# asmekal/ubdvss

Measured on AMD Instinct MI355X. Metric: images/sec (512x512) fwd+CCL, higher is better.
Workload: dtype f32; 1 GPU; configs[1]: batch=32 512x512x3 fp32 forward + CCL postprocess per GPU (stripe-textured rectangle images, random-init weights); batch_per_gpu=32, parallelism=replicas x1, no collective

## Files before the change

### ubdvss_amd/csrc/api.hip

```cpp
#include <stdarg.h>
#include <stddef.h>
#include <stdlib.h>
#include <string.h>
#include <thread>
#include "common.h"

static thread_local char g_err[512] = "";

void ubd_set_error(const char *fmt, ...)
{
    va_list ap;
    va_start(ap, fmt);
    vsnprintf(g_err, sizeof(g_err), fmt, ap);
    va_end(ap);
}

extern "C" const char *ubd_last_error(void) { return g_err; }
extern "C" int ubd_abi_version(void) { return UBD_ABI_VERSION; }
#ifndef UBD_BUILD_ID
#define UBD_BUILD_ID "unknown"
#endif
extern "C" int ubd_host_memcpy_mt(void *dst, const void *src, size_t n, int threads)
{
    if (threads < 1) threads = 1;
    if (threads > 16) threads = 16;
    if (n < ((size_t)1 << 20)) threads = 1;
    const size_t piece = ((n + threads - 1) / threads + 4095) & ~(size_t)4095;
    std::thread th[16];
    int started = 0;
    size_t done_to = n < piece ? n : piece;
    for (int t = 1; t < threads; ++t) {
        const size_t a = (size_t)t * piece;
        if (a >= n) break;
        const size_t len = n - a < piece ? n - a : piece;
        try {
            th[started] = std::thread([=] { memcpy((char *)dst + a, (const char *)src + a, len); });
            ++started;
        } catch (...) {
            memcpy((char *)dst + a, (const char *)src + a, n - a);
            break;
        }
    }
    memcpy(dst, src, done_to);
    for (int t = 0; t < started; ++t) th[t].join();
    return 0;
}
extern "C" const char *ubd_build_id(void) { return UBD_BUILD_ID; }

#ifdef UBD_STAMPS
static struct { const char *kernel; ubd_stamp_buf buf; int sel0, sel1; } g_stamps[] = {
    {"stem23"}, {"stem123"}, {"wino"}, {"wino6"}, {"sep123_16"}, {"dilconv16s"}, {"sepb16"}, {"sep_bwd"}, {"dil_wgrad16"}, {"postprocess"}, {"loss"},
};
extern "C" int ubd_debug_set_stamps(const char *kernel, void *buf, size_t capacity_words, int sel0, int sel1)
{
    for (auto &e : g_stamps)
        if (kernel && strcmp(kernel, e.kernel) == 0) {
            e.buf = {(unsigned long long *)buf, buf ? capacity_words : 0};
            e.sel0 = sel0; e.sel1 = sel1;
            return 0;
        }
    UBD_REQUIRE(false, "ubd_debug_set_stamps: no kernel family named %s", kernel ? kernel : "(null)");
}
ubd_stamp_buf ubd_stamps_for(const char *kernel, int sel0, int sel1)
{
    for (const auto &e : g_stamps)
        if (strcmp(kernel, e.kernel) == 0) return e.sel0 == sel0 && e.sel1 == sel1 ? e.buf : ubd_stamp_buf{nullptr, 0};
    return {nullptr, 0};
}
#endif

static const char ANY[] = "", NUMBER[] = "#";
struct env_switch { const char *name; size_t field; const char *value; int set; };
#define SW(name, field, value, set) {name, offsetof(ubd_handle, field), value, set}
static const env_switch ENV_SWITCHES[] = {
    SW("UBD_DILCONV", use_wino, "direct", 0), SW("UBD_DILCONV", wino_x6, "direct", 0), SW("UBD_DILCONV", wino_x6, "wino32", 0),
    SW("UBD_WINO6_LAYOUT", wino6_natural, "natural", 1),
    SW("UBD_STEM", fuse_stem, "fused", UBD_STEM_FUSED23), SW("UBD_STEM", fuse_force, "fused", 1),
    SW("UBD_STEM", fuse_stem, "fused123", UBD_STEM_FUSED123), SW("UBD_STEM", fuse_force, "fused123", 1),
    SW("UBD_STEM", fuse_stem, "unfused", UBD_STEM_SEPARATE),
    SW("UBD_TEST_NUM_CUS", num_cus, NUMBER, 0),
    SW("UBD_DILBWD", split_dilbwd, "split", 1), SW("UBD_DILBWD", no_pair_dilbwd, "pair8", 1),
    SW("UBD_SEPBWD", split_sepbwd32, "split", 1),
    SW("UBD_STEM16", split_stem16, "split", 1), SW("UBD_STEM16", split_stem16, "fused12", 2),
    SW("UBD_PP_GLOBAL", pp_global, ANY, 1), SW("UBD_PP_SPLIT", pp_split, ANY, 1), SW("UBD_PP_POISON", pp_poison, ANY, 1),
    SW("UBD_PP_SERIAL_TAIL", pp_serial_tail, ANY, 1), SW("UBD_PP_THREADS_512", pp_threads_512, ANY, 1),
    SW("UBD_HEADBWD", split_headbwd, "split", 1),
    SW("UBD_SEPB16_X", sepb_x_regs, "regs", 1),
    SW("UBD_REDUCE", chain_reduce, "batched", 0),
    SW("UBD_LOSS", loss_chain, "chain", 1),
    SW("UBD_DILCONV16", direct_dil16, "direct", 1),
};
#undef SW

extern "C" int ubd_create(const ubd_config *cfg, ubd_handle **out)
{
    UBD_REQUIRE(cfg && out, "ubd_create: null argument");
    UBD_REQUIRE(cfg->c_in == 1 || cfg->c_in == 3, "ubd_create: c_in must be 1 (grey) or 3, got %d", cfg->c_in);
    UBD_REQUIRE(cfg->n_classes >= 0 && cfg->n_classes <= UBD_MAX_CLASSES, "ubd_create: n_classes %d out of range [0,%d]", cfg->n_classes, UBD_MAX_CLASSES);
    UBD_REQUIRE(cfg->dtype == UBD_F32 || cfg->dtype == UBD_BF16 || cfg->dtype == UBD_F16, "ubd_create: bad dtype %d", cfg->dtype);
    int ndev = 0;
    hipError_t e = hipGetDeviceCount(&ndev);
    UBD_REQUIRE(e == hipSuccess && ndev > 0, "ubd_create: no HIP device visible (%s); this library has no CPU fallback", hipGetErrorString(e));
    int dev = 0;
    UBD_CHECK_HIP(hipGetDevice(&dev));
    hipDeviceProp_t prop;
    UBD_CHECK_HIP(hipGetDeviceProperties(&prop, dev));
    UBD_REQUIRE(strncmp(prop.gcnArchName, "gfx950", 6) == 0, "ubd_create: device arch %s is not gfx950; this library is built for MI355X only", prop.gcnArchName);

    ubd_handle *h = (ubd_handle *)calloc(1, sizeof(ubd_handle));
    UBD_REQUIRE(h, "ubd_create: out of host memory");
    h->cfg = *cfg;
    h->k_out = 1 + cfg->n_classes;
    h->num_cus = prop.multiProcessorCount;
    h->use_wino = h->wino_x6 = h->chain_reduce = 1;
    h->fuse_stem = cfg->fml_compatible != 0 ? UBD_STEM_FUSED123 : UBD_STEM_SEPARATE;
    for (const env_switch &sw : ENV_SWITCHES) {
        const char *e = getenv(sw.name);
        if (!e) continue;
        int *field = (int *)((char *)h + sw.field);
        if (sw.value == NUMBER) { if (atoi(e) > 0) *field = atoi(e); }
        else if (sw.value == ANY || strcmp(e, sw.value) == 0) *field = sw.set;
    }
    { const char *s = getenv("UBD_STEM"); if (s && strcmp(s, "cold123") == 0 && cfg->fml_compatible != 0) { h->fuse_stem = UBD_STEM_COLD123; h->fuse_force = 1; } }
    size_t off = 0;
    int cin = cfg->c_in;
    for (int s = 0; s < 3; ++s) {
        h->off_sep_dw[s] = off; off += (size_t)9 * cin;
        h->off_sep_pw[s] = off; off += (size_t)cin * UBD_C;
        h->off_sep_b[s] = off;  off += UBD_C;
        cin = UBD_C;
    }
    for (int k = 0; k < UBD_NUM_DIL; ++k) {
        h->off_dil_k[k] = off; off += (size_t)9 * UBD_C * UBD_C;
        h->off_dil_b[k] = off; off += UBD_C;
    }
    h->off_head_k = off; off += (size_t)UBD_C * h->k_out;
    h->off_head_b = off; off += h->k_out;
    h->n_params = off;
    *out = h;
    return 0;
}

extern "C" void ubd_destroy(ubd_handle *h)
{
    if (h && h->comm) ubd_comm_destroy(h);
    free(h);
}

extern "C" size_t ubd_param_count(const ubd_handle *h) { return h ? h->n_params : 0; }
extern "C" int ubd_num_cus(const ubd_handle *h) { return h ? h->num_cus : 0; }
```

### ubdvss_amd/csrc/common.h

```cpp
#pragma once
#include <hip/hip_runtime.h>
#include <stdint.h>
#include <stdio.h>
#include <string.h>
#include <type_traits>
#include "../../include/ubd.h"
#include "stem_plan.h"
#include "stamps.h"

#define UBD_C 24
#define UBD_NUM_DIL 6

struct ubd_comm;
struct ubd_handle {
    ubd_config cfg;
    ubd_comm *comm;
    int k_out;
    size_t off_sep_dw[3], off_sep_pw[3], off_sep_b[3];
    size_t off_dil_k[UBD_NUM_DIL], off_dil_b[UBD_NUM_DIL];
    size_t off_head_k, off_head_b;
    size_t n_params;
    int num_cus;
    int pp_lds_attr_set;
    int fuse_force;
    int split_headbwd;
    int no_pair_dilbwd;
    int split_dilbwd;
    int split_stem16;
    int pp_global, pp_split, pp_poison, pp_serial_tail, pp_threads_512;
    int sepb_x_regs;
    int split_sepbwd32;
    int chain_reduce;
    int direct_dil16;
    int fuse_stem;
    int use_wino;
    int loss_chain;
    int wino_x6;
    int wino6_natural;
};

static const int UBD_DILATIONS[UBD_NUM_DIL] = {1, 2, 4, 8, 16, 1};

#if defined(__HIPCC__)
__device__ __forceinline__ int ubd_xcd_tile(int L, int total)
{
    return (total & 7) == 0 ? (L & 7) * (total >> 3) + (L >> 3) : L;
}
#endif

#if defined(__HIPCC__)
__device__ __forceinline__ void ubd_glds16_at(const void *gsrc, unsigned lds_dst)
{
    unsigned keep;
    asm volatile("s_mov_b32 %0, m0\n\ts_mov_b32 m0, %2\n\ts_nop 0\n\tglobal_load_lds_dwordx4 %1, off\n\ts_mov_b32 m0, %0"
                 : "=&s"(keep) : "v"(gsrc), "s"(lds_dst) : "memory");
}
__device__ __forceinline__ void ubd_glds16_sbase(const void *base_uniform, unsigned voff, unsigned lds_dst)
{
    unsigned keep;
    asm volatile("s_mov_b32 %0, m0\n\ts_mov_b32 m0, %3\n\ts_nop 0\n\tglobal_load_lds_dwordx4 %1, %2\n\ts_mov_b32 m0, %0"
                 : "=&s"(keep) : "v"(voff), "s"(base_uniform), "s"(lds_dst) : "memory");
}
__device__ __forceinline__ void ubd_blds16(__amdgpu_buffer_rsrc_t rsrc, unsigned voff, unsigned lds_dst)
{
    unsigned keep;
    asm volatile("s_mov_b32 %0, m0\n\ts_mov_b32 m0, %3\n\ts_nop 0\n\tbuffer_load_dwordx4 %1, %2, 0 offen lds\n\ts_mov_b32 m0, %0"
                 : "=&s"(keep) : "v"(voff), "s"(rsrc), "s"(lds_dst) : "memory");
}
__device__ __forceinline__ void ubd_blds4(__amdgpu_buffer_rsrc_t rsrc, unsigned voff, unsigned lds_dst)
{
    unsigned keep;
    asm volatile("s_mov_b32 %0, m0\n\ts_mov_b32 m0, %3\n\ts_nop 0\n\tbuffer_load_dword %1, %2, 0 offen lds\n\ts_mov_b32 m0, %0"
                 : "=&s"(keep) : "v"(voff), "s"(rsrc), "s"(lds_dst) : "memory");
}
__device__ __forceinline__ float ubd_relu_cap(float x, float cap) { return __builtin_amdgcn_fmed3f(x, 0.f, cap); }
__device__ __forceinline__ unsigned ubd_lds_addr(const void *lds_generic)
{
    return (unsigned)__builtin_amdgcn_readfirstlane((int)(unsigned)(size_t)(__attribute__((address_space(3))) const char *)lds_generic);
}
__device__ __forceinline__ void ubd_glds16(const void *gsrc, const void *lds_generic) { ubd_glds16_at(gsrc, ubd_lds_addr(lds_generic)); }
#endif

#if defined(__HIPCC__)
template <int D, int NMAX> struct ubd_magic24 {
    static constexpr int find_sh()
    {
        for (int sh = 8; sh < 24; ++sh) {
            const long m = (1L << sh) / D + 1;
            if (m * NMAX >= (1L << 24)) continue;
            bool ok = true;
            for (long n = 0; n < NMAX && ok; ++n) ok = ((n * m) >> sh) == n / D;
            if (ok) return sh;
        }
        return -1;
    }
    static constexpr int sh = find_sh();
    static_assert(sh > 0, "no 24-bit magic number for this divisor / range");
    static constexpr unsigned m = (1u << sh) / D + 1;
};

__device__ __forceinline__ int ubd_mul24(int a, int b) { return __mul24(a, b); }
template <int D, int NMAX> __device__ __forceinline__ int ubd_div24(int n) { return (int)(__umul24((unsigned)n, ubd_magic24<D, NMAX>::m) >> ubd_magic24<D, NMAX>::sh); }
struct ubd_tile_decoder {
    unsigned tiles_x, tiles_y, mx, my, total;
    bool fast;
    __device__ __forceinline__ void init(int tx_, int ty_, int total_)
    {
        tiles_x = (unsigned)tx_; tiles_y = (unsigned)ty_; total = (unsigned)total_;
        mx = 0xFFFFFFFFu / tiles_x + 1u;
        my = 0xFFFFFFFFu / tiles_y + 1u;
        const unsigned dmax = tiles_x > tiles_y ? tiles_x : tiles_y;
        fast = (unsigned long long)total * dmax < 0x100000000ull;
    }
    __device__ __forceinline__ unsigned div_x(unsigned v) const { return fast ? (tiles_x == 1u ? v : __umulhi(v, mx)) : v / tiles_x; }
    __device__ __forceinline__ unsigned div_y(unsigned v) const { return fast ? (tiles_y == 1u ? v : __umulhi(v, my)) : v / tiles_y; }
    __device__ __forceinline__ void decode(int L, int &tx, int &ty, int &img) const
    {
        const unsigned tile = (unsigned)ubd_xcd_tile(L, (int)total);
        const unsigned r = div_x(tile);
        tx = (int)(tile - r * tiles_x);
        const unsigned im = div_y(r);
        ty = (int)(r - im * tiles_y);
        img = (int)im;
    }
};
#endif

void ubd_set_error(const char *fmt, ...);

#define UBD_CHECK_HIP(expr)                                                              \
    do {                                                                                 \
        hipError_t _e = (expr);                                                          \
        if (_e != hipSuccess) {                                                          \
            ubd_set_error("%s:%d: %s failed: %s", __FILE__, __LINE__, #expr,             \
                          hipGetErrorString(_e));                                        \
            return 1;                                                                    \
        }                                                                                \
    } while (0)

#define UBD_REQUIRE(cond, ...)                                                           \
    do {                                                                                 \
        if (!(cond)) {                                                                   \
            ubd_set_error(__VA_ARGS__);                                                  \
            return 2;                                                                    \
        }                                                                                \
    } while (0)

static inline size_t ubd_align_up(size_t v, size_t a) { return (v + a - 1) / a * a; }

static inline bool ubd_pixels_by_lds_dma(bool f32_in, float sub, float div, int H, int W, int c_in, size_t limit, const void *x)
{
    return f32_in && sub == 0.f && div == 1.f && (size_t)H * W * c_in * 4 < limit && ((uintptr_t)x & 15) == 0;
}
static inline bool ubd_head_in_epilogue(const ubd_handle *h) { return h->k_out == 1 && h->off_head_b == h->off_head_k + UBD_C; }
template <int V> using ubd_int = std::integral_constant<int, V>;
template <typename F> static inline void ubd_dispatch_bool(bool b, F f) { if (b) f(std::true_type{}); else f(std::false_type{}); }
template <typename F> static inline void ubd_dispatch_input(int c_in, bool u8, F f)
{
    if (c_in == 1) { if (u8) f(ubd_int<1>{}, ubd_int<1>{}); else f(ubd_int<1>{}, ubd_int<0>{}); }
    else { if (u8) f(ubd_int<3>{}, ubd_int<1>{}); else f(ubd_int<3>{}, ubd_int<0>{}); }
}

#define UBD_DIL_FRAG_FLOATS (9 * 6 * 2 * 64)
#define UBD_SEP_FRAG_FLOATS (6 * 2 * 64)
#define UBD_SEP_DW_FLOATS (9 * 6 * 64)
#define UBD_WINO_FRAG_FLOATS (16 * 6 * 64 * 2)
#define UBD_FWD_DIRECT_FLOATS (3 * (UBD_SEP_FRAG_FLOATS + UBD_SEP_DW_FLOATS) + UBD_NUM_DIL * UBD_DIL_FRAG_FLOATS)
#define UBD_WINO6_FRAG_U32 (16 * 2 * 3 * 64 * 4)
#define UBD_FWD_WINO6_OFF (UBD_FWD_DIRECT_FLOATS + UBD_NUM_DIL * UBD_WINO_FRAG_FLOATS)
#define UBD_FWD_FRAG_FLOATS (UBD_FWD_WINO6_OFF + UBD_NUM_DIL * UBD_WINO6_FRAG_U32)

struct ubd_fwd_layout {
    size_t off_tickets;
    size_t off_wfrag;
    size_t off_a1, off_a2;
    size_t off_b[2];
    size_t off_acts[7];
    size_t total;
};

bool ubd_comm_fused(const ubd_handle *h);
bool ubd_comm_global_loss(const ubd_handle *h);
int ubd_comm_rank(const ubd_handle *h);
enum { UBD_RED_F64 = 0, UBD_RED_I32 = 1, UBD_RED_U32 = 2 };
int ubd_comm_allreduce_raw(ubd_handle *h, void *buf, size_t count, int kind, hipStream_t st);
int ubd_comm_allgather_u32(ubd_handle *h, const unsigned *send_one, unsigned *recv_world, hipStream_t st);
extern "C" int ubd_comm_world(const ubd_handle *h);
int ubd_comm_begin_tail(ubd_handle *h, float *grads, hipStream_t st);
int ubd_comm_finish(ubd_handle *h, float *grads, hipStream_t st);
void ubd_fwd_layout_compute(const ubd_handle *h, int n, int H, int W, int training, ubd_fwd_layout *L);
struct pp_lds_args;
int ubd_forward_impl(ubd_handle *h, const float *params, const void *images, int in_dtype, int preprocessing,
                     int n, int H, int W, float *logits, char *ws, const ubd_fwd_layout &L, hipStream_t st, bool inference = false,
                     const pp_lds_args *pp_job = nullptr);
int ubd_pp_fill_job(ubd_handle *hd, const float *logits, int n, int map_h, int map_w, float logit_threshold, int scale, float min_area,
                    int32_t *binary_map, int32_t *quads, int32_t *classes, int32_t *counts, int cap, void *workspace,
                    size_t workspace_bytes, int threads, pp_lds_args *job);
void ubd_launch_dilconv(const ubd_handle *h, int epi, const float *frag, const float *aux, int dilation,
                        const float *in, float *out, int n, int H4, int W4, hipStream_t st);
int ubd_grid_for(long waves_needed, int num_cus, int waves_per_block, int blocks_per_cu);
int ubd_loss_impl(const float *logits, int k_out, const int32_t *y_true, long npix, float *loss, float *dlogits,
                  char *ws, hipStream_t st, ubd_handle *h = nullptr, bool prezeroed = false);
size_t ubd_loss_zero_bytes(void);
extern "C" size_t ubd_loss_workspace_bytes(const ubd_handle *h, int n, int map_h, int map_w);
void ubd_launch_pack_wino(const ubd_handle *h, const float *params, float *out, int transpose, hipStream_t st);
void ubd_launch_dilconv_wino(const ubd_handle *h, int epi, const float *frag, const void *aux, int aux_dtype, int dilation,
                             const float *in, float *out, int n, int H4, int W4, hipStream_t st, const float *head = nullptr);
void ubd_launch_pack_wino6(const ubd_handle *h, const float *params, unsigned *out, hipStream_t st);
void ubd_launch_dilconv_wino6(const ubd_handle *h, int epi, const unsigned *frag, const float *bias, int dilation,
                              const float *in, float *out, int n, int H4, int W4, hipStream_t st, const float *head = nullptr,
                              int lay_in = 1, int lay_out = 1);
void ubd_launch_pack_direct(const ubd_handle *h, const float *params, float *wfrag, hipStream_t st);
size_t ubd_forward16_workspace_bytes(int n, int H, int W);
int ubd_pack16_workspace(ubd_handle *h, const float *params, char *ws, size_t ws_bytes, hipStream_t st);
int ubd_forward16(ubd_handle *h, const float *params, const void *images, int in_dtype, int preprocessing, int n, int H, int W,
                  float *logits, char *ws, size_t ws_bytes, hipStream_t st);
#define UBD_SEP16_READY_U32 (2 * 10 * 64 * 4)
#define UBD_DIL16_FRAG_U32 (7 * 2 * 64 * 4)
void ubd_launch_dilconv16(const ubd_handle *h, int epi, const unsigned *frag, const float *bias, const void *mask, int d,
                          const void *in, void *out, int n, int H4, int W4, hipStream_t st, float *logits3 = nullptr);
void ubd_launch_pack16(const ubd_handle *h, const float *params, unsigned *out, int transpose, hipStream_t st);
struct ubd_fwd16_layout { size_t off_wfrag32, off_wfrag16, off_a1, off_a2, off_acts[7], total; };
void ubd_fwd16_layout_compute(int n, int H, int W, int training, ubd_fwd16_layout *L);
int ubd_forward16_layout(ubd_handle *h, const float *params, const void *images, int in_dtype, int preprocessing, int n, int H,
                         int W, float *logits, char *ws, const ubd_fwd16_layout &L, hipStream_t st, bool inference = false);
```

### ubdvss_amd/csrc/forward.hip

```cpp
#include "common.h"

typedef float f32x4 __attribute__((ext_vector_type(4)));
typedef float f32x2 __attribute__((ext_vector_type(2)));
typedef unsigned int u32x4 __attribute__((ext_vector_type(4)));
typedef unsigned int u32x2 __attribute__((ext_vector_type(2)));

#include "pack.h"
__global__ void pack_weights_kernel(const float *__restrict__ params, float *__restrict__ wfrag, pack_args a)
{
    pack_weights_body(params, wfrag, a, (int)(blockIdx.x * blockDim.x + threadIdx.x), (int)(gridDim.x * blockDim.x));
}

__device__ __forceinline__ void store_tile_relu(float *__restrict__ y, size_t row_base_elems, int x0, int ow,
                                                int lane, f32x4 acc0, f32x4 acc1, float b0, float b1)
{
    const int co = lane & 15, q = lane >> 4;
    const unsigned long long rp = (unsigned long long)(y + (row_base_elems + (size_t)x0) * UBD_C);
    const unsigned rlo = (unsigned)__builtin_amdgcn_readfirstlane((int)(unsigned)rp);
    const unsigned rhi = (unsigned)__builtin_amdgcn_readfirstlane((int)(unsigned)(rp >> 32));
    float *rowp = (float *)(((unsigned long long)rhi << 32) | rlo);
    int npx = ow - x0 < 16 ? ow - x0 : 16;
    npx = npx < 0 ? 0 : npx;
    const unsigned bytes = (unsigned)__builtin_amdgcn_readfirstlane(npx * UBD_C * 4);
    __amdgpu_buffer_rsrc_t rs = __builtin_amdgcn_make_buffer_rsrc((void *)rowp, 0, (int)bytes, 0x00020000);
    const unsigned base = (unsigned)(4 * q) * (UBD_C * 4u) + (unsigned)co * 4u;
    const unsigned base1 = co < 8 ? base + 64u : 0x40000000u;
#pragma unroll
    for (int r = 0; r < 4; ++r) {
        __builtin_amdgcn_raw_buffer_store_b32(__builtin_bit_cast(unsigned, fmaxf(acc0[r] + b0, 0.f)), rs, (int)(base + r * 96u), 0, 0);
        __builtin_amdgcn_raw_buffer_store_b32(__builtin_bit_cast(unsigned, fmaxf(acc1[r] + b1, 0.f)), rs, (int)(base1 + r * 96u), 0, 0);
    }
}

__device__ __forceinline__ void store_tile_relu_t(float *__restrict__ y, size_t row_base_elems, int x0, int ow,
                                                  int lane, f32x4 acc0, f32x4 acc1, f32x4 bA, f32x4 bB)
{
    const int i = lane & 15, q = lane >> 4;
    const unsigned long long rp = (unsigned long long)(y + (row_base_elems + (size_t)x0) * UBD_C);
    const unsigned rlo = (unsigned)__builtin_amdgcn_readfirstlane((int)(unsigned)rp);
    const unsigned rhi = (unsigned)__builtin_amdgcn_readfirstlane((int)(unsigned)(rp >> 32));
    float *rowp = (float *)(((unsigned long long)rhi << 32) | rlo);
    int npx = ow - x0 < 16 ? ow - x0 : 16;
    npx = npx < 0 ? 0 : npx;
    const unsigned bytes = (unsigned)__builtin_amdgcn_readfirstlane(npx * UBD_C * 4);
    __amdgpu_buffer_rsrc_t rs = __builtin_amdgcn_make_buffer_rsrc((void *)rowp, 0, (int)bytes, 0x00020000);
    const unsigned base = (unsigned)i * (UBD_C * 4u) + 16u * (unsigned)q;
    const unsigned base1 = q < 2 ? base + 64u : 0x40000000u;
    f32x4 o0, o1;
#pragma unroll
    for (int r = 0; r < 4; ++r) { o0[r] = fmaxf(acc0[r] + bA[r], 0.f); o1[r] = fmaxf(acc1[r] + bB[r], 0.f); }
    __builtin_amdgcn_raw_buffer_store_b128(__builtin_bit_cast(u32x4, o0), rs, (int)base, 0, 0);
    __builtin_amdgcn_raw_buffer_store_b128(__builtin_bit_cast(u32x4, o1), rs, (int)base1, 0, 0);
}

__device__ __forceinline__ void store_tile_relu_nb(float *__restrict__ y, size_t row_base_elems, int x0, int ow,
                                                   int lane, f32x4 acc0, f32x4 acc1, bool drop = false ,
                                                   int l2p = 0)
{
    const int i = lane & 15, q = lane >> 4;
    const unsigned long long rp = (unsigned long long)(y + row_base_elems * UBD_C);
    const unsigned rlo = (unsigned)__builtin_amdgcn_readfirstlane((int)(unsigned)rp);
    const unsigned rhi = (unsigned)__builtin_amdgcn_readfirstlane((int)(unsigned)(rp >> 32));
    float *rowp = (float *)(((unsigned long long)rhi << 32) | rlo);
    const unsigned bytes = (unsigned)__builtin_amdgcn_readfirstlane(ow * UBD_C * 4);
    __amdgpu_buffer_rsrc_t rs = __builtin_amdgcn_make_buffer_rsrc((void *)rowp, 0, (int)bytes, 0x00020000);
    const int x = x0 + i, r = x & ((1 << l2p) - 1), wr = ow & ((1 << l2p) - 1);
    const int pos = r * (ow >> l2p) + (r < wr ? r : wr) + (x >> l2p);
    const unsigned base = (drop || x >= ow) ? 0x40000000u : (unsigned)pos * (UBD_C * 4u) + 16u * (unsigned)q;
    const unsigned base1 = (q < 2 && !drop) ? base + 64u : 0x40000000u;
    const float cap = __builtin_inff();
    f32x4 o0, o1;
#pragma unroll
    for (int r = 0; r < 4; ++r) { o0[r] = ubd_relu_cap(acc0[r], cap); o1[r] = ubd_relu_cap(acc1[r], cap); }
    __builtin_amdgcn_raw_buffer_store_b128(__builtin_bit_cast(u32x4, o0), rs, (int)base, 0, 0);
    __builtin_amdgcn_raw_buffer_store_b128(__builtin_bit_cast(u32x4, o1), rs, (int)base1, 0, 0);
}

__device__ __forceinline__ void store_tile_masked(float *__restrict__ y, const float (&mk)[8],
                                                  size_t row_base_elems, int x0, int ow, int lane, f32x4 acc0, f32x4 acc1)
{
    const int co = lane & 15, q = lane >> 4;
#pragma unroll
    for (int r = 0; r < 4; ++r) {
        int px = x0 + 4 * q + r;
        if (px < ow) {
            const size_t e = (row_base_elems + (size_t)px) * UBD_C;
            y[e + co] = mk[r] > 0.f ? acc0[r] : 0.f;
            if (co < 8) y[e + 16 + co] = mk[4 + r] > 0.f ? acc1[r] : 0.f;
        }
    }
}

template <int CIN, int STRIDE> struct sep_cfg {
    static constexpr int TH = (CIN == UBD_C) ? (STRIDE == 2 ? 4 : 8) : 16;
    static constexpr int PH = (TH - 1) * STRIDE + 3;
    static constexpr int PW = 15 * STRIDE + 3;
    static constexpr int PS = CIN;
    static constexpr int CHUNKS = (CIN == UBD_C) ? PH * PW * 6 : 0;
    static constexpr int ELEMS = PH * PW * CIN;
    static constexpr int BUF_FLOATS = (CIN == UBD_C) ? (CHUNKS + 255) / 256 * 256 * 4 : (ELEMS + 3) / 4 * 4;
    static constexpr int STAGE_REGS = (CIN == UBD_C) ? 1 : (ELEMS + 255) / 256;
};

template <int CIN, int STRIDE, int IN_U8>
__global__ __launch_bounds__(256, (CIN == UBD_C) ? (STRIDE == 1 ? 3 : 2) : 5) void sepconv_kernel(const void *__restrict__ xin, float *__restrict__ y,
                                                      const float *__restrict__ frag,
                                                      const float *__restrict__ bias, int n, int H, int W, int OH,
                                                      int OW, int pad_lo, float pre_sub, float pre_div)
{
    using C = sep_cfg<CIN, STRIDE>;
    constexpr int CPL = (CIN == UBD_C) ? 6 : 1;
    constexpr int NBUF = (CIN == UBD_C) ? 2 : 1;
    __shared__ __attribute__((aligned(16))) float patch_mem[NBUF * C::BUF_FLOATS];
    const int lane = threadIdx.x & 63, wid = __builtin_amdgcn_readfirstlane((int)(threadIdx.x >> 6));
    const int i = lane & 15, q = lane >> 4;
    const float *pwfrag = frag;
    const float *dwlane = frag + UBD_SEP_FRAG_FLOATS;

    const int tiles_x = (OW + 15) >> 4, tiles_y = (OH + C::TH - 1) / C::TH;
    const int total = n * tiles_y * tiles_x;

    float dwk[9][CPL];
    float pwf[CPL][2];
#pragma unroll
    for (int s = 0; s < CPL; ++s) {
        const int ch = (CIN == UBD_C) ? (s < 4 ? 4 * q + s : 16 + 2 * q + (s - 4)) : 0;
        const int src_lane = (CIN == UBD_C) ? 16 * (ch / 6) + i : lane, ss = (CIN == UBD_C) ? ch % 6 : s;
#pragma unroll
        for (int t = 0; t < 9; ++t) dwk[t][s] = dwlane[(t * 6 + ss) * 64 + src_lane];
        pwf[s][0] = pwfrag[(ss * 2 + 0) * 64 + src_lane];
        pwf[s][1] = pwfrag[(ss * 2 + 1) * 64 + src_lane];
    }
    const f32x4 bA = *(const f32x4 *)(bias + 4 * q);
    const f32x4 bB = q < 2 ? *(const f32x4 *)(bias + 16 + 4 * q) : f32x4{0.f, 0.f, 0.f, 0.f};
    const int cb = (q < CIN) ? q : 0;

    ubd_tile_decoder tdec;
    tdec.init(tiles_x, tiles_y, total);
    auto tile_coords = [&](int tile, int &img, int &oy0, int &ox0) {
        int tx, ty;
        tdec.decode(tile, tx, ty, img);
        oy0 = ty * C::TH; ox0 = tx * 16;
    };
    constexpr int ROUNDS = (CIN == UBD_C) ? (C::CHUNKS + 255) / 256 : 1;
    int dma_rel[ROUNDS];
    if constexpr (CIN == UBD_C) {
#pragma unroll
        for (int rd = 0; rd < ROUNDS; ++rd) {
            int c = rd * 256 + wid * 64 + lane;
            c = c < C::CHUNKS ? c : C::CHUNKS - 1;
            const int pix = c / 6, sp = c - pix * 6;
            const int pr = pix / C::PW, pc = pix - pr * C::PW;
            int part = sp + 3 * ((pc >> 3) & 1);
            part = part >= 6 ? part - 6 : part;
            dma_rel[rd] = ((pr * W + pc) * UBD_C + part * 4) * 4;
        }
    }
    auto dma_tile = [&](int tile, float *buf) {
        int img, oy0, ox0;
        tile_coords(tile, img, oy0, ox0);
        const int ix0 = ox0 * STRIDE - pad_lo, iy0 = oy0 * STRIDE - pad_lo;
        const char *src = (const char *)xin;
        const bool interior = (iy0 >= 0) && (ix0 >= 0) && (iy0 + C::PH <= H) && (ix0 + C::PW <= W);
        if (interior) {
            const char *origin = src + (((size_t)img * H + iy0) * W + ix0) * (UBD_C * sizeof(float));
#pragma unroll
            for (int rd = 0; rd < ROUNDS; ++rd)
                __builtin_amdgcn_global_load_lds((const __attribute__((address_space(1))) void *)(origin + dma_rel[rd]),
                                                 (__attribute__((address_space(3))) void *)(buf + (rd * 256 + wid * 64) * 4), 16, 0, 0);
            return;
        }
        __amdgpu_buffer_rsrc_t rsrc = __builtin_amdgcn_make_buffer_rsrc((void *)(src + (size_t)img * H * W * (UBD_C * sizeof(float))), 0,
                                                                        (int)((unsigned)H * W * (unsigned)(UBD_C * sizeof(float))), 0x00020000);
#pragma unroll
        for (int rd = 0; rd < ROUNDS; ++rd) {
            const int cbase = rd * 256 + wid * 64;
            int c = cbase + lane;
            c = c < C::CHUNKS ? c : C::CHUNKS - 1;
            const int pix = c / 6, sp = c - pix * 6;
            const int pr = pix / C::PW, pc = pix - pr * C::PW;
            int part = sp + 3 * ((pc >> 3) & 1);
            part = part >= 6 ? part - 6 : part;
            const int gy = iy0 + pr, gx = ix0 + pc;
            const unsigned off = (unsigned)gx < (unsigned)W ? (unsigned)(((gy * W + gx) * UBD_C + part * 4) * (int)sizeof(float)) : 0x80000000u;
            __builtin_amdgcn_raw_ptr_buffer_load_lds(rsrc, (__attribute__((address_space(3))) void *)(buf + cbase * 4), 16, (int)off, 0, 0, 0);
        }
    };
    int ld_rel[C::STAGE_REGS];
    if constexpr (CIN != UBD_C) {
#pragma unroll
        for (int k = 0; k < C::STAGE_REGS; ++k) {
            int e = k * 256 + threadIdx.x;
            e = e < C::ELEMS ? e : C::ELEMS - 1;
            const int pix = e / CIN, ch = e - pix * CIN;
            const int pr = pix / C::PW, pc = pix - pr * C::PW;
            ld_rel[k] = (pr * W + pc) * CIN + ch;
        }
    }
    auto load_regs = [&](int tile, unsigned (&st)[C::STAGE_REGS]) {
        int img, oy0, ox0;
        tile_coords(tile, img, oy0, ox0);
        const int ix0 = ox0 * STRIDE - pad_lo, iy0 = oy0 * STRIDE - pad_lo;
        const bool interior = (iy0 >= 0) && (ix0 >= 0) && (iy0 + C::PH <= H) && (ix0 + C::PW <= W);
        if (interior) {
            const size_t origin = (((size_t)img * H + iy0) * W + ix0) * CIN;
#pragma unroll
            for (int k = 0; k < C::STAGE_REGS; ++k) {
                if constexpr (IN_U8) st[k] = ((const unsigned char *)xin)[origin + ld_rel[k]];
                else st[k] = ((const unsigned *)xin)[origin + ld_rel[k]];
            }
            return;
        }
        const int WC = W * CIN;
        const unsigned char *img8 = (const unsigned char *)xin + (size_t)img * H * WC * ((IN_U8) ? 1 : 4);
#pragma unroll
        for (int k = 0; k < C::STAGE_REGS; ++k) {
            int e = k * 256 + threadIdx.x;
            e = e < C::ELEMS ? e : C::ELEMS - 1;
            const int pr = e / (C::PW * CIN), pf = e - pr * (C::PW * CIN);
            const int gy = min(max(iy0 + pr, 0), H - 1), gf = min(max(ix0 * CIN + pf, 0), WC - 1);
            const unsigned off = (unsigned)(gy * WC + gf);
            if constexpr (IN_U8) st[k] = img8[off];
            else st[k] = ((const unsigned *)img8)[off];
        }
#pragma unroll
        for (int k = 0; k < C::STAGE_REGS; ++k) {
            int e = k * 256 + threadIdx.x;
            e = e < C::ELEMS ? e : C::ELEMS - 1;
            const int pr = e / (C::PW * CIN), pf = e - pr * (C::PW * CIN);
            const bool inside = (unsigned)(iy0 + pr) < (unsigned)H && (unsigned)(ix0 * CIN + pf) < (unsigned)WC;
            st[k] = inside ? st[k] : ((IN_U8) ? 0x100u : __builtin_bit_cast(unsigned, pre_sub));
        }
    };

    int tile = blockIdx.x;
    if (tile >= total) return;
    unsigned stage[C::STAGE_REGS];
    if constexpr (CIN == UBD_C) dma_tile(tile, patch_mem);
    else load_regs(tile, stage);

    for (int it = 0;; ++it) {
        float *patch = patch_mem + ((CIN == UBD_C) ? (it & 1) * C::BUF_FLOATS : 0);
        int img, oy0, ox0;
        tile_coords(tile, img, oy0, ox0);
        const int nxt = tile + gridDim.x;
        const bool has_next = (CIN == UBD_C) && nxt < total;
        if constexpr (CIN == UBD_C) {
            constexpr int NSTORE = (C::TH / 4) * 2;
            if (it == 0) asm volatile("s_waitcnt vmcnt(0)" ::: "memory");
            else if constexpr (NSTORE == 8) asm volatile("s_waitcnt vmcnt(8)" ::: "memory");
            else if constexpr (NSTORE == 4) asm volatile("s_waitcnt vmcnt(4)" ::: "memory");
            else { static_assert(NSTORE == 2, "counted vmcnt"); asm volatile("s_waitcnt vmcnt(2)" ::: "memory"); }
            __builtin_amdgcn_s_barrier();
            if (has_next) dma_tile(nxt, patch_mem + ((it + 1) & 1) * C::BUF_FLOATS);
        } else {
            __builtin_amdgcn_s_barrier();
#pragma unroll
            for (int k = 0; k < C::STAGE_REGS; ++k) {
                const int e = k * 256 + threadIdx.x;
                if (e < C::ELEMS) {
                    if constexpr (IN_U8) patch[e] = stage[k] > 255u ? 0.f : ((float)stage[k] - pre_sub) / pre_div;
                    else patch[e] = (__builtin_bit_cast(float, stage[k]) - pre_sub) / pre_div;
                }
            }
            __builtin_amdgcn_s_waitcnt(0xC07F);
            __builtin_amdgcn_s_barrier();
            if (has_next) load_regs(nxt, stage);
        }

        if constexpr (CIN == UBD_C && STRIDE == 1) {
            constexpr int RW = C::TH / 4;
            const int rb = wid * RW;
            float dwv[RW][6];
#pragma unroll
            for (int o = 0; o < RW; ++o)
#pragma unroll
                for (int s = 0; s < 6; ++s) dwv[o][s] = 0.f;
#pragma unroll
            for (int yy = 0; yy < RW + 2; ++yy) {
                f32x4 v4[3];
                f32x2 v2[3];
#pragma unroll
                for (int kx = 0; kx < 3; ++kx) {
                    const int pcol = i + kx;
                    const float *p = patch + ((rb + yy) * C::PW + pcol) * C::PS;
                    const int rot = 3 * ((pcol >> 3) & 1);
                    int s4 = q + rot, s2 = 4 + (q >> 1) + rot;
                    s4 = s4 >= 6 ? s4 - 6 : s4; s2 = s2 >= 6 ? s2 - 6 : s2;
                    v4[kx] = *(const f32x4 *)(p + 4 * s4);
                    v2[kx] = *(const f32x2 *)(p + 4 * s2 + 2 * (q & 1));
                }
#pragma unroll
                for (int o = 0; o < RW; ++o) {
                    const int ky = yy - o;
                    if (ky < 0 || ky > 2) continue;
#pragma unroll
                    for (int kx = 0; kx < 3; ++kx) {
                        const int t = ky * 3 + kx;
                        dwv[o][0] = fmaf(v4[kx][0], dwk[t][0], dwv[o][0]);
                        dwv[o][1] = fmaf(v4[kx][1], dwk[t][1], dwv[o][1]);
                        dwv[o][2] = fmaf(v4[kx][2], dwk[t][2], dwv[o][2]);
                        dwv[o][3] = fmaf(v4[kx][3], dwk[t][3], dwv[o][3]);
                        dwv[o][4] = fmaf(v2[kx][0], dwk[t][4], dwv[o][4]);
                        dwv[o][5] = fmaf(v2[kx][1], dwk[t][5], dwv[o][5]);
                    }
                }
                if (yy >= 2) {
                    const int o = yy - 2, oy = oy0 + rb + o;
                    f32x4 acc0 = {0.f, 0.f, 0.f, 0.f}, acc1 = {0.f, 0.f, 0.f, 0.f};
#pragma unroll
                    for (int s = 0; s < 6; ++s) {
                        acc0 = __builtin_amdgcn_mfma_f32_16x16x4f32(pwf[s][0], dwv[o][s], acc0, 0, 0, 0);
                        acc1 = __builtin_amdgcn_mfma_f32_16x16x4f32(pwf[s][1], dwv[o][s], acc1, 0, 0, 0);
                    }
                    store_tile_relu_t(y, ((size_t)img * OH + oy) * OW, ox0, oy < OH ? OW : 0, lane, acc0, acc1, bA, bB);
                }
            }
        } else {
        for (int r = wid; r < C::TH; r += 4) {
            const int oy = oy0 + r;
            float dwv[CPL];
#pragma unroll
            for (int s = 0; s < CPL; ++s) dwv[s] = 0.f;
#pragma unroll
            for (int ky = 0; ky < 3; ++ky) {
#pragma unroll
                for (int kx = 0; kx < 3; ++kx) {
                    const int pcol = i * STRIDE + kx;
                    const float *p = patch + ((r * STRIDE + ky) * C::PW + pcol) * C::PS;
                    const int t = ky * 3 + kx;
                    if constexpr (CIN == UBD_C) {
                        const int rot = 3 * ((pcol >> 3) & 1);
                        int s4 = q + rot, s2 = 4 + (q >> 1) + rot;
                        s4 = s4 >= 6 ? s4 - 6 : s4; s2 = s2 >= 6 ? s2 - 6 : s2;
                        const f32x4 v4 = *(const f32x4 *)(p + 4 * s4);
                        const f32x2 v2 = *(const f32x2 *)(p + 4 * s2 + 2 * (q & 1));
                        dwv[0] = fmaf(v4[0], dwk[t][0], dwv[0]);
                        dwv[1] = fmaf(v4[1], dwk[t][1], dwv[1]);
                        dwv[2] = fmaf(v4[2], dwk[t][2], dwv[2]);
                        dwv[3] = fmaf(v4[3], dwk[t][3], dwv[3]);
                        dwv[4] = fmaf(v2[0], dwk[t][4], dwv[4]);
                        dwv[5] = fmaf(v2[1], dwk[t][5], dwv[5]);
                    } else {
                        dwv[0] = fmaf(p[cb], dwk[t][0], dwv[0]);
                    }
                }
            }
            f32x4 acc0 = {0.f, 0.f, 0.f, 0.f}, acc1 = {0.f, 0.f, 0.f, 0.f};
#pragma unroll
            for (int s = 0; s < CPL; ++s) {
                acc0 = __builtin_amdgcn_mfma_f32_16x16x4f32(pwf[s][0], dwv[s], acc0, 0, 0, 0);
                acc1 = __builtin_amdgcn_mfma_f32_16x16x4f32(pwf[s][1], dwv[s], acc1, 0, 0, 0);
            }
            store_tile_relu_t(y, ((size_t)img * OH + oy) * OW, ox0, oy < OH ? OW : 0, lane, acc0, acc1, bA, bB);
        }
        }
        if (!has_next) break;
        tile = nxt;
    }
}

#include "pp_lds.h"
#include "stem23.h"
#include "stem123.h"

struct a_frags {
    f32x4 v4[9];
    f32x2 v2[9];
};

__device__ __forceinline__ void dil_load(a_frags &a, __amdgpu_buffer_rsrc_t rsrc, unsigned oob, int tile,
                                         int tiles_x, int h, int w, int d, int lane)
{
    const int i = lane & 15, q = lane >> 4;
    const int xt = (int)((unsigned)tile % (unsigned)tiles_x);
    const int rowid = (int)((unsigned)tile / (unsigned)tiles_x);
    const int yy = (int)((unsigned)rowid % (unsigned)h);
    const int px = xt * 16 + i;
#pragma unroll
    for (int ky = 0; ky < 3; ++ky) {
        const int iy = yy + (ky - 1) * d;
        const bool rok = (iy >= 0) && (iy < h);
#pragma unroll
        for (int kx = 0; kx < 3; ++kx) {
            const int ix = px + (kx - 1) * d;
            const bool ok = rok && (ix >= 0) && (ix < w);
            const unsigned byte_off = (unsigned)((rowid + (ky - 1) * d) * w + ix) * (unsigned)(UBD_C * 4);
            const unsigned o4 = ok ? byte_off + 16u * q : oob;
            const unsigned o2 = ok ? byte_off + 64u + 8u * q : oob;
            u32x4 r4 = __builtin_amdgcn_raw_buffer_load_b128(rsrc, (int)o4, 0, 0);
            u32x2 r2 = __builtin_amdgcn_raw_buffer_load_b64(rsrc, (int)o2, 0, 0);
            a.v4[ky * 3 + kx] = __builtin_bit_cast(f32x4, r4);
            a.v2[ky * 3 + kx] = __builtin_bit_cast(f32x2, r2);
        }
    }
}

template <int EPI>
__global__ __launch_bounds__(256, 2) void dilconv_f32_kernel(const float *__restrict__ x, float *__restrict__ y,
                                                             const float *__restrict__ wfrag,
                                                             const float *__restrict__ bias, int n, int h, int w,
                                                             int d, unsigned in_bytes)
{
    const int lane = threadIdx.x & 63;
    const int i = lane & 15;
    float wr[9][6][2];
#pragma unroll
    for (int t = 0; t < 9; ++t)
#pragma unroll
        for (int j = 0; j < 6; ++j) {
            wr[t][j][0] = wfrag[((t * 6 + j) * 2 + 0) * 64 + lane];
            wr[t][j][1] = wfrag[((t * 6 + j) * 2 + 1) * 64 + lane];
        }
    float b0 = 0.f, b1 = 0.f;
    if constexpr (EPI == 0) { b0 = bias[i]; b1 = (i < 8) ? bias[16 + i] : 0.f; }

    const int tiles_x = (w + 15) >> 4;
    const int total = n * h * tiles_x;
    const int xcd = blockIdx.x & 7;
    const int nblk_x = (gridDim.x + 7 - xcd) >> 3;
    const int chunk = (total + 7) >> 3;
    const int t_begin = xcd * chunk;
    const int t_end = (t_begin + chunk < total) ? t_begin + chunk : total;
    const int stride = nblk_x * 4;
    int tile = t_begin + (int)(blockIdx.x >> 3) * 4 + __builtin_amdgcn_readfirstlane((int)(threadIdx.x >> 6));
    if (tile >= t_end) return;

    __amdgpu_buffer_rsrc_t rsrc = __builtin_amdgcn_make_buffer_rsrc((void *)x, 0, (int)in_bytes, 0x00020000);
    const unsigned oob = in_bytes;

    auto compute_store = [&](const a_frags &a, int tl) {
        f32x4 acc0 = {0.f, 0.f, 0.f, 0.f}, acc1 = {0.f, 0.f, 0.f, 0.f};
        float mk[8];
        if constexpr (EPI == 1) {
            const int co = lane & 15, q = lane >> 4;
            const int xt0 = (int)((unsigned)tl % (unsigned)tiles_x);
            const int rid = (int)((unsigned)tl / (unsigned)tiles_x);
#pragma unroll
            for (int r = 0; r < 4; ++r) {
                const int opx = xt0 * 16 + 4 * q + r;
                const size_t e = ((size_t)rid * w + (size_t)(opx < w ? opx : 0)) * UBD_C;
                mk[r] = bias[e + co];
                mk[4 + r] = bias[e + 16 + (co & 7)];
            }
        }
#pragma unroll
        for (int t = 0; t < 9; ++t) {
#pragma unroll
            for (int j = 0; j < 4; ++j) {
                acc0 = __builtin_amdgcn_mfma_f32_16x16x4f32(a.v4[t][j], wr[t][j][0], acc0, 0, 0, 0);
                acc1 = __builtin_amdgcn_mfma_f32_16x16x4f32(a.v4[t][j], wr[t][j][1], acc1, 0, 0, 0);
            }
#pragma unroll
            for (int j = 0; j < 2; ++j) {
                acc0 = __builtin_amdgcn_mfma_f32_16x16x4f32(a.v2[t][j], wr[t][4 + j][0], acc0, 0, 0, 0);
                acc1 = __builtin_amdgcn_mfma_f32_16x16x4f32(a.v2[t][j], wr[t][4 + j][1], acc1, 0, 0, 0);
            }
        }
        const int xt = (int)((unsigned)tl % (unsigned)tiles_x);
        const int rowid = (int)((unsigned)tl / (unsigned)tiles_x);
        if constexpr (EPI == 0) store_tile_relu(y, (size_t)rowid * w, xt * 16, w, lane, acc0, acc1, b0, b1);
        else store_tile_masked(y, mk, (size_t)rowid * w, xt * 16, w, lane, acc0, acc1);
    };

    a_frags A0, A1;
    const int t_last = t_end - 1;
    dil_load(A0, rsrc, oob, tile, tiles_x, h, w, d, lane);
    for (;;) {
        int nxt = tile + stride;
        dil_load(A1, rsrc, oob, nxt < t_last ? nxt : t_last, tiles_x, h, w, d, lane);
        compute_store(A0, tile);
        tile = nxt;
        if (tile >= t_end) break;
        nxt = tile + stride;
        dil_load(A0, rsrc, oob, nxt < t_last ? nxt : t_last, tiles_x, h, w, d, lane);
        compute_store(A1, tile);
        tile = nxt;
        if (tile >= t_end) break;
    }
}

__global__ __launch_bounds__(256) void head_kernel(const float *__restrict__ x, float *__restrict__ logits,
                                                   const float *__restrict__ hk, const float *__restrict__ hb,
                                                   long npix, int k_out)
{
    __shared__ float s_k[UBD_C * (UBD_MAX_CLASSES + 1)];
    __shared__ float s_b[UBD_MAX_CLASSES + 1];
    for (int t = threadIdx.x; t < UBD_C * k_out; t += blockDim.x) s_k[t] = hk[t];
    for (int t = threadIdx.x; t < k_out; t += blockDim.x) s_b[t] = hb[t];
    __syncthreads();
    for (long p = (long)blockIdx.x * blockDim.x + threadIdx.x; p < npix; p += (long)gridDim.x * blockDim.x) {
        const f32x4 *px = (const f32x4 *)(x + p * UBD_C);
        float v[UBD_C];
#pragma unroll
        for (int c4 = 0; c4 < 6; ++c4) {
            f32x4 t = px[c4];
            v[c4 * 4 + 0] = t[0]; v[c4 * 4 + 1] = t[1]; v[c4 * 4 + 2] = t[2]; v[c4 * 4 + 3] = t[3];
        }
        for (int ko = 0; ko < k_out; ++ko) {
            float acc = 0.f;
#pragma unroll
            for (int c = 0; c < UBD_C; ++c) acc = fmaf(v[c], s_k[c * k_out + ko], acc);
            logits[p * k_out + ko] = acc + s_b[ko];
        }
    }
}

static size_t act_bytes(const ubd_handle *, long n, long hh, long ww) { return (size_t)(n * hh * ww) * UBD_C * sizeof(float); }

void ubd_fwd_layout_compute(const ubd_handle *h, int n, int H, int W, int training, ubd_fwd_layout *L)
{
    const size_t wf = (size_t)UBD_FWD_FRAG_FLOATS * sizeof(float);
    size_t off = 0;
    L->off_wfrag = off; off += ubd_align_up(wf, 256);
    L->off_tickets = off; off += 256;
    const size_t a = ubd_align_up(act_bytes(h, n, H / 2, W / 2), 256);
    const size_t b = ubd_align_up(act_bytes(h, n, H / 4, W / 4), 256);
    L->off_a1 = off; off += a;
    L->off_a2 = off; off += a;
    if (training) {
        for (int k = 0; k < 7; ++k) { L->off_acts[k] = off; off += b; }
        L->off_b[0] = L->off_acts[0]; L->off_b[1] = L->off_acts[1];
    } else {
        L->off_b[0] = off; off += b;
        L->off_b[1] = off; off += b;
        for (int k = 0; k < 7; ++k) L->off_acts[k] = L->off_b[k & 1];
    }
    L->total = off;
}

extern "C" size_t ubd_forward_workspace_bytes(const ubd_handle *h, int n, int height, int width)
{
    if (h && h->cfg.dtype != UBD_F32) return ubd_forward16_workspace_bytes(n, height, width);
    ubd_fwd_layout L;
    ubd_fwd_layout_compute(h, n, height, width, 0, &L);
    return L.total;
}

int ubd_grid_for(long waves_needed, int num_cus, int waves_per_block, int blocks_per_cu)
{
    long blocks = (waves_needed + waves_per_block - 1) / waves_per_block;
    long cap = (long)num_cus * blocks_per_cu;
    if (blocks > cap) blocks = cap;
    if (blocks < 1) blocks = 1;
    return (int)blocks;
}

template <int CIN, int STRIDE>
static void launch_sep(const ubd_handle *h, const void *x, int in_u8, float *y, const float *frag, const float *bias,
                       int n, int H, int W, int OH, int OW, int pad_lo, float sc, float sh, hipStream_t st)
{
    const int th = sep_cfg<CIN, STRIDE>::TH;
    const int tiles = n * ((OH + th - 1) / th) * ((OW + 15) / 16);
    const int per_cu = (CIN == UBD_C) ? (STRIDE == 1 ? 3 : 2) : 5;
    int grid = h->num_cus * per_cu;
    if (grid > tiles || CIN != UBD_C) grid = tiles;
    ubd_dispatch_bool(in_u8 != 0, [&](auto u8) {
        hipLaunchKernelGGL((sepconv_kernel<CIN, STRIDE, decltype(u8)::value>), dim3(grid), dim3(256), 0, st, x, y, frag, bias, n, H, W, OH, OW, pad_lo, sc, sh);
    });
}

void ubd_launch_pack_direct(const ubd_handle *h, const float *params, float *wfrag, hipStream_t st)
{
    pack_args pa;
    for (int s = 0; s < 3; ++s) { pa.off_sep_dw[s] = h->off_sep_dw[s]; pa.off_sep_pw[s] = h->off_sep_pw[s]; }
    for (int k = 0; k < UBD_NUM_DIL; ++k) pa.off_dil_k[k] = h->off_dil_k[k];
    pa.c_in = h->cfg.c_in;
    hipLaunchKernelGGL(pack_weights_kernel, dim3(64), dim3(256), 0, st, params, wfrag, pa);
}

static void launch_pack(const ubd_handle *h, const float *params, float *wfrag, hipStream_t st)
{
    ubd_launch_pack_direct(h, params, wfrag, st);
    if (h->use_wino) ubd_launch_pack_wino(h, params, wfrag + UBD_FWD_DIRECT_FLOATS, 0, st);
    if (h->wino_x6) ubd_launch_pack_wino6(h, params, (unsigned *)(wfrag + UBD_FWD_WINO6_OFF), st);
}

void ubd_launch_dilconv(const ubd_handle *h, int epi, const float *frag, const float *aux, int dilation,
                        const float *in, float *out, int n, int H4, int W4, hipStream_t st)
{
    const unsigned in_bytes = (unsigned)((size_t)n * H4 * W4 * UBD_C * 4);
    const long tiles = (long)n * H4 * ((W4 + 15) / 16);
    int grid = ubd_grid_for(tiles, h->num_cus, 4, 2);
    grid = (grid + 7) / 8 * 8;
    if (epi == 0)
        hipLaunchKernelGGL(dilconv_f32_kernel<0>, dim3(grid), dim3(256), 0, st, in, out, frag, aux, n, H4, W4, dilation, in_bytes);
    else
        hipLaunchKernelGGL(dilconv_f32_kernel<1>, dim3(grid), dim3(256), 0, st, in, out, frag, aux, n, H4, W4, dilation, in_bytes);
}

static void launch_dil(const ubd_handle *h, const float *params, const float *wfrag, int k, const float *in, float *out,
                       int n, int H4, int W4, hipStream_t st, int lay_in = 1, int lay_out = 1)
{
    if (h->wino_x6) {
        ubd_launch_dilconv_wino6(h, 0, (const unsigned *)(wfrag + UBD_FWD_WINO6_OFF) + (size_t)k * UBD_WINO6_FRAG_U32, params + h->off_dil_b[k],
                                 UBD_DILATIONS[k], in, out, n, H4, W4, st, nullptr, lay_in, lay_out);
        return;
    }
    if (h->use_wino) {
        ubd_launch_dilconv_wino(h, 0, wfrag + UBD_FWD_DIRECT_FLOATS + (size_t)k * UBD_WINO_FRAG_FLOATS, params + h->off_dil_b[k], UBD_F32,
                                UBD_DILATIONS[k], in, out, n, H4, W4, st);
        return;
    }
    const int per_sep = UBD_SEP_FRAG_FLOATS + UBD_SEP_DW_FLOATS;
    const float *dfrag = wfrag + 3 * per_sep;
    ubd_launch_dilconv(h, 0, dfrag + (size_t)k * UBD_DIL_FRAG_FLOATS, params + h->off_dil_b[k], UBD_DILATIONS[k], in, out, n, H4, W4, st);
}

extern "C" int ubd_pack_weights(ubd_handle *h, const float *params, void *workspace, size_t workspace_bytes, void *stream)
{
    UBD_REQUIRE(h && params && workspace, "ubd_pack_weights: null argument");
    if (h->cfg.dtype != UBD_F32) return ubd_pack16_workspace(h, params, (char *)workspace, workspace_bytes, (hipStream_t)stream);
    ubd_fwd_layout L;
    ubd_fwd_layout_compute(h, 1, 4, 4, 0, &L);
    UBD_REQUIRE(workspace_bytes >= L.off_a1, "ubd_pack_weights: workspace too small");
    launch_pack(h, params, (float *)((char *)workspace + L.off_wfrag), (hipStream_t)stream);
    UBD_CHECK_HIP(hipMemsetAsync((char *)workspace + L.off_tickets, 0, 256, (hipStream_t)stream));
    UBD_CHECK_HIP(hipGetLastError());
    return 0;
}

extern "C" int ubd_dilated_layer(ubd_handle *h, const float *params, int layer, const void *in, void *out, int n,
                                 int map_h, int map_w, const void *workspace, void *stream)
{
    UBD_REQUIRE(h && params && in && out && workspace, "ubd_dilated_layer: null argument");
    UBD_REQUIRE(layer >= 0 && layer < UBD_NUM_DIL, "ubd_dilated_layer: layer %d out of range", layer);
    UBD_REQUIRE(h->cfg.dtype == UBD_F32, "ubd_dilated_layer: only UBD_F32 in this build");
    UBD_REQUIRE((size_t)n * map_h * map_w * UBD_C * 4 <= (1ull << 30), "ubd_dilated_layer: tensor too large (activation bytes must not exceed 2^30)");
    launch_dil(h, params, (const float *)workspace, layer, (const float *)in, (float *)out, n, map_h, map_w, (hipStream_t)stream);
    UBD_CHECK_HIP(hipGetLastError());
    return 0;
}

static int check_forward_input(int n, int H, int W, int in_dtype)
{
    UBD_REQUIRE(n > 0 && H > 0 && W > 0 && (H % 4) == 0 && (W % 4) == 0, "ubd_forward: height and width must be positive multiples of 4 (got %d x %d)", H, W);
    UBD_REQUIRE((in_dtype & ~UBD_IN_PREPACKED) == UBD_IN_F32 || (in_dtype & ~UBD_IN_PREPACKED) == UBD_IN_U8, "ubd_forward: bad in_dtype %d", in_dtype);
    return 0;
}

template <bool COLD>
static void launch_stem123(const ubd_handle *h, const float *params, const void *images, bool u8, float *a3, const float *sf0, const float *sf1,
                           const float *sf2, int n, int H, int W, float sc, float sh, long units, int *ticket, const pp_lds_args *job, int a3_l2p,
                           hipStream_t st)
{
    const int H2 = H / 2, W2 = W / 2, H4 = H / 4, W4 = W / 4;
    const int grid = units < h->num_cus ? (int)units : h->num_cus;
    pp_lds_args pj;
    memset(&pj, 0, sizeof(pj));
    if (job) pj = *job;
    const float *b0 = params + h->off_sep_b[0], *b1 = params + h->off_sep_b[1], *b2 = params + h->off_sep_b[2];
    const bool plain = ubd_pixels_by_lds_dma(!u8, sc, sh, H, W, h->cfg.c_in, 1ull << 30, images);
    ubd_dispatch_input(h->cfg.c_in, u8, [&](auto cin, auto in_u8) {
        auto launch = [&](auto pl) {
            hipLaunchKernelGGL((stem123_kernel<decltype(cin)::value, decltype(in_u8)::value, decltype(pl)::value, COLD>), dim3(grid), dim3(s23_cfg::NT), 0, st,
                               images, a3, sf0, b0, sf1, b1, sf2, b2, n, H, W, H2, W2, H4, W4, sc, sh, ticket, pj, a3_l2p
                               UBD_STAMP_ARG(COLD ? "" : "stem123"));
        };
        if constexpr (decltype(in_u8)::value == 0) { if (plain) return launch(ubd_int<1>{}); }
        launch(ubd_int<0>{});
    });
}

int ubd_forward_impl(ubd_handle *h, const float *params, const void *images, int in_dtype, int preprocessing,
                     int n, int H, int W, float *logits, char *ws, const ubd_fwd_layout &L, hipStream_t st, bool inference,
                     const pp_lds_args *pp_job)
{
    UBD_REQUIRE(h->cfg.dtype == UBD_F32, "ubd_forward: only UBD_F32 activations are implemented in this build");
    const bool prepacked = (in_dtype & UBD_IN_PREPACKED) != 0;
    in_dtype &= ~UBD_IN_PREPACKED;
    if (int rc = check_forward_input(n, H, W, in_dtype)) return rc;
    UBD_REQUIRE(!(in_dtype == UBD_IN_U8 && h->cfg.c_in == UBD_C), "ubd_forward: u8 input needs c_in 1 or 3");
    const int H2 = H / 2, W2 = W / 2, H4 = H / 4, W4 = W / 4;
    UBD_REQUIRE((size_t)n * H4 * W4 * UBD_C * 4 <= (1ull << 30), "ubd_forward: batch too large for 32-bit buffer offsets; split the batch");
    float *wfrag = (float *)(ws + L.off_wfrag);
    float *a1 = (float *)(ws + L.off_a1), *a2 = (float *)(ws + L.off_a2);

    if (!prepacked) {
        launch_pack(h, params, wfrag, st);
        UBD_CHECK_HIP(hipMemsetAsync(ws + L.off_tickets, 0, 256, st));
    }

    const int per_sep = UBD_SEP_FRAG_FLOATS + UBD_SEP_DW_FLOATS;
    const float *sf0 = wfrag, *sf1 = wfrag + per_sep, *sf2 = wfrag + 2 * per_sep;
    const int pad_s2 = h->cfg.fml_compatible ? 1 : 0;
    float sc = 0.f, sh = 1.f;
    if (preprocessing == UBD_PRE_MOBILENET) { sc = 127.5f; sh = 127.5f; }
    const int u8 = in_dtype == UBD_IN_U8;
    float *cur = (float *)(ws + L.off_acts[0]);
    static_assert(UBD_STEM_STRIP_ROWS == s23_cfg::TH3, "stem_plan.h counts the strips the stem kernels walk");
    const ubd_stem_plan plan = ubd_plan_stem(h->fuse_stem, h->fuse_force != 0, h->cfg.fml_compatible != 0, h->num_cus, n, H, inference, pp_job != nullptr);
    UBD_REQUIRE(!plan.job_without_strips, "ubd_forward: a postprocess job needs the fused stem kernel (internal error)");
    const bool one_kernel = plan.form == UBD_STEM_FORM_STRIPS || plan.form == UBD_STEM_FORM_COLD;
    static const int phase_lay[UBD_NUM_DIL + 1] = {2, 4, 1, 1, 1, 2, 1};
    const bool phase_major = h->wino_x6 && !h->wino6_natural && one_kernel;
    const int a3_l2p = phase_major ? 1 : 0;
    int *ticket = (int *)(ws + L.off_tickets);
    if (plan.form == UBD_STEM_FORM_COLD)
        launch_stem123<true>(h, params, images, u8, cur, sf0, sf1, sf2, n, H, W, sc, sh, plan.strips * (W4 <= 16 ? 1 : 1 + (W4 - 16 + 14) / 15),
                             ticket, nullptr, a3_l2p, st);
    else if (plan.form == UBD_STEM_FORM_STRIPS)
        launch_stem123<false>(h, params, images, u8, cur, sf0, sf1, sf2, n, H, W, sc, sh, plan.strips, ticket, pp_job, a3_l2p, st);
    else if (h->cfg.c_in == 1)
        launch_sep<1, 2>(h, images, u8, a1, sf0, params + h->off_sep_b[0], n, H, W, H2, W2, pad_s2, sc, sh, st);
    else
        launch_sep<3, 2>(h, images, u8, a1, sf0, params + h->off_sep_b[0], n, H, W, H2, W2, pad_s2, sc, sh, st);
    if (plan.form == UBD_STEM_FORM_L1_STEM23) {
        const int grid = plan.strips < h->num_cus ? (int)plan.strips : h->num_cus;
        ubd_dispatch_bool(pad_s2 != 0, [&](auto pad) {
            hipLaunchKernelGGL(stem23_kernel<decltype(pad)::value>, dim3(grid), dim3(s23_cfg::NT), 0, st, a1, cur, sf1, params + h->off_sep_b[1], sf2,
                               params + h->off_sep_b[2], n, H2, W2, H4, W4, pad_s2 UBD_STAMP_ARG("stem23"));
        });
    } else if (plan.form == UBD_STEM_FORM_SEPARATE) {
        launch_sep<UBD_C, 1>(h, a1, 0, a2, sf1, params + h->off_sep_b[1], n, H2, W2, H2, W2, 1, 0.f, 1.f, st);
        launch_sep<UBD_C, 2>(h, a2, 0, cur, sf2, params + h->off_sep_b[2], n, H2, W2, H4, W4, pad_s2, 0.f, 1.f, st);
    }

    const bool fuse_head = inference && h->use_wino && ubd_head_in_epilogue(h);
    for (int k = 0; k < UBD_NUM_DIL; ++k) {
        float *nxt = (float *)(ws + L.off_acts[k + 1]);
        if (fuse_head && k == UBD_NUM_DIL - 1) {
            if (h->wino_x6)
                ubd_launch_dilconv_wino6(h, 2, (const unsigned *)(wfrag + UBD_FWD_WINO6_OFF) + (size_t)k * UBD_WINO6_FRAG_U32, params + h->off_dil_b[k],
                                         UBD_DILATIONS[k], cur, logits, n, H4, W4, st, params + h->off_head_k, phase_major ? phase_lay[k] : 1, 1);
            else
                ubd_launch_dilconv_wino(h, 2, wfrag + UBD_FWD_DIRECT_FLOATS + (size_t)k * UBD_WINO_FRAG_FLOATS, params + h->off_dil_b[k], UBD_F32,
                                        UBD_DILATIONS[k], cur, logits, n, H4, W4, st, params + h->off_head_k);
            UBD_CHECK_HIP(hipGetLastError());
            return 0;
        }
        launch_dil(h, params, wfrag, k, cur, nxt, n, H4, W4, st, phase_major ? phase_lay[k] : 1, phase_major ? phase_lay[k + 1] : 1);
        cur = nxt;
    }
    const long npix = (long)n * H4 * W4;
    int hgrid = (int)((npix + 255) / 256);
    if (hgrid > h->num_cus * 8) hgrid = h->num_cus * 8;
    hipLaunchKernelGGL(head_kernel, dim3(hgrid), dim3(256), 0, st, cur, logits, params + h->off_head_k, params + h->off_head_b, npix, h->k_out);
    UBD_CHECK_HIP(hipGetLastError());
    return 0;
}

static int forward_f32(ubd_handle *h, const float *params, const void *images, int in_dtype, int preprocessing, int n, int H, int W, float *logits,
                       void *workspace, size_t workspace_bytes, void *stream, const pp_lds_args *pp_job)
{
    ubd_fwd_layout L;
    ubd_fwd_layout_compute(h, n, H, W, 0, &L);
    UBD_REQUIRE(workspace_bytes >= L.total, "ubd_forward: workspace too small (%zu < %zu)", workspace_bytes, L.total);
    return ubd_forward_impl(h, params, images, in_dtype, preprocessing, n, H, W, logits, (char *)workspace, L, (hipStream_t)stream, true, pp_job);
}

extern "C" int ubd_forward(ubd_handle *h, const float *params, const void *images, int in_dtype, int preprocessing,
                           int n, int height, int width, float *logits, void *workspace, size_t workspace_bytes,
                           void *stream)
{
    UBD_REQUIRE(h && params && images && logits && workspace, "ubd_forward: null argument");
    if (h->cfg.dtype != UBD_F32) {
        if (int rc = check_forward_input(n, height, width, in_dtype)) return rc;
        return ubd_forward16(h, params, images, in_dtype, preprocessing, n, height, width, logits, (char *)workspace, workspace_bytes, (hipStream_t)stream);
    }
    return forward_f32(h, params, images, in_dtype, preprocessing, n, height, width, logits, workspace, workspace_bytes, stream, nullptr);
}

extern "C" int ubd_forward_postprocess(ubd_handle *h, const float *params, const void *images, int in_dtype, int preprocessing,
                                       int n, int height, int width, float *logits, void *workspace, size_t workspace_bytes,
                                       const float *pp_logits, int pp_n, int pp_map_h, int pp_map_w, float logit_threshold, int scale,
                                       float min_area, int32_t *binary_map, int32_t *quads, int32_t *classes, int32_t *counts, int cap,
                                       void *pp_workspace, size_t pp_workspace_bytes, void *stream)
{
    UBD_REQUIRE(h && params && images && logits && workspace, "ubd_forward_postprocess: null argument");
    UBD_REQUIRE(pp_logits != logits, "ubd_forward_postprocess: the logits being postprocessed must not be the buffer this call writes");
    if (h->cfg.dtype == UBD_F32 && n > 0 && height > 0 && (height % 4) == 0 &&
        ubd_plan_stem(h->fuse_stem, h->fuse_force != 0, h->cfg.fml_compatible != 0, h->num_cus, n, height, true, true).form == UBD_STEM_FORM_STRIPS) {
        pp_lds_args job;
        const int fits = ubd_pp_fill_job(h, pp_logits, pp_n, pp_map_h, pp_map_w, logit_threshold, scale, min_area, binary_map, quads, classes,
                                         counts, cap, pp_workspace, pp_workspace_bytes,
                                         s23_cfg::NT, &job);
        if (fits < 0) return 1;
        if (fits == 1) return forward_f32(h, params, images, in_dtype, preprocessing, n, height, width, logits, workspace, workspace_bytes, stream, &job);
    }
    int rc = ubd_postprocess(h, pp_logits, pp_n, pp_map_h, pp_map_w, logit_threshold, scale, min_area, binary_map, quads, classes, counts, cap,
                             pp_workspace, pp_workspace_bytes, stream);
    if (rc) return rc;
    return ubd_forward(h, params, images, in_dtype, preprocessing, n, height, width, logits, workspace, workspace_bytes, stream);
}
```

### ubdvss_amd/csrc/stem123.h

```cpp
#pragma once
#include "split3.h"

__device__ __forceinline__ int s123_slot(int c, int col) { return c < 4 ? (c ^ ((col >> 2) & 1)) : 4 + ((c - 4) ^ ((col >> 3) & 1)); }

template <int CIN> struct s123_cfg {
    using B = s23_cfg;
    static constexpr int NT = B::NT, NW = B::NW;
    static constexpr int AC = B::LC + 1;
    static constexpr int XH = 2 * B::PH + 1, XW = 2 * AC + 1;
    static constexpr int XE = XH * XW * CIN;
    static constexpr int XREGS = (XE + NT - 1) / NT;
    static constexpr int XCH = ((XW + 1) * CIN + 3) / 4;
    static constexpr int XS = XCH * 4;
    static constexpr int XP_FLOATS = XH * XS;
    static constexpr int A1_FLOATS = B::PH * B::PW * UBD_C;
    static constexpr int NPIX = B::PH * AC;
    static constexpr int UNITS = (NPIX + 15) / 16;
    static constexpr int UPW = (UNITS + NW - 1) / NW;
    static constexpr int W1_FLOATS = 64 * 12 + 64 + 4;
    static constexpr int LUT_FLOATS = 256;
    static constexpr int PWS_U32 = 2 * 3 * 64 * 4;
    static constexpr int STEM_FLOATS = A1_FLOATS + B::L2_FLOATS + XP_FLOATS + 2 * PWS_U32 + B::W3DW_FLOATS + B::CARRY_FLOATS + W1_FLOATS + LUT_FLOATS;
    static constexpr int PP_FLOATS = (PP_LDS_MAX_BYTES + 3) / 4;
    static constexpr int SMEM_FLOATS = STEM_FLOATS > PP_FLOATS ? STEM_FLOATS : PP_FLOATS;
    static_assert(XCH <= 64 && (A1_FLOATS % 4) == 0 && (B::L2_FLOATS % 4) == 0, "patch rows are single 16-byte-aligned DMA pieces");
};

template <int CIN, int IN_U8, int PLAIN, bool COLD = false>
__global__ __launch_bounds__(s23_cfg::NT, 1) void stem123_kernel(const void *__restrict__ xin, float *__restrict__ y,
                                                                const float *__restrict__ frag1, const float *__restrict__ bias1,
                                                                const float *__restrict__ frag2, const float *__restrict__ bias2,
                                                                const float *__restrict__ frag3, const float *__restrict__ bias3,
                                                                int n, int H, int W, int H2, int W2, int H4, int W4,
                                                                float pre_sub, float pre_div, int *__restrict__ ticket, pp_lds_args pj,
                                                                int a3_l2p
                                                                UBD_STAMP_PARAM)
{
    using C = s23_cfg;
    using X = s123_cfg<CIN>;
    __shared__ __attribute__((aligned(16))) float smem[X::SMEM_FLOATS];
#define S123_BLOCK_STAMP(k) UBD_STAMP_RT(threadIdx.x == 0 && (k) < 32, (size_t)gridDim.x * 8 * 16 * 8 + (size_t)blockIdx.x * 32 + (k))
    S123_BLOCK_STAMP(0);
    if (pj.n > 0) {
        for (int im = (int)blockIdx.x; im < pj.n; im += (int)gridDim.x) {
            pp_image_lds<C::NT, true>((int *)smem, pj, im);
            __syncthreads();
        }
    }
    S123_BLOCK_STAMP(1);
    const int Dc = ((W4 + 15) >> 4) >= 3 ? 1 : 4 - ((W4 + 15) >> 4);
    const int njob = pj.n > 0 ? (pj.n < (int)gridDim.x ? pj.n : (int)gridDim.x) : 0;
    auto ticket_ls = [&](int k) { return k < njob * Dc ? k : k + ((int)gridDim.x - njob) * Dc; };
    int t0_early = 0;
    if (!COLD && threadIdx.x == 0 && (int)blockIdx.x < njob) t0_early = __hip_atomic_fetch_add(ticket, Dc, __ATOMIC_RELAXED, __HIP_MEMORY_SCOPE_AGENT);
    float *a1p = smem;
    float *l2 = a1p + X::A1_FLOATS;
    float *xp = l2 + C::L2_FLOATS;
    unsigned *pws = (unsigned *)(xp + X::XP_FLOATS);
    float *w3dw = (float *)(pws + 2 * X::PWS_U32);
    float *carry_buf = w3dw + C::W3DW_FLOATS;
    const int lane = threadIdx.x & 63, wid = __builtin_amdgcn_readfirstlane((int)(threadIdx.x >> 6));
    const int i = lane & 15, q = lane >> 4;

    float dwk2[9][6];
#pragma unroll
    for (int s = 0; s < 6; ++s) {
        const int ch = s < 4 ? 4 * q + s : 16 + 2 * q + (s - 4);
        const int src_lane = 16 * (ch / 6) + i, ss = ch % 6;
#pragma unroll
        for (int t = 0; t < 9; ++t) dwk2[t][s] = frag2[UBD_SEP_FRAG_FLOATS + (t * 6 + ss) * 64 + src_lane];
    }
    auto pw_split = [&](const unsigned *tab, f32x4 v4, f32x2 v2, f32x4 &acc0, f32x4 &acc1) {
        const u32x4 *w = (const u32x4 *)tab + lane;
        const f32x4 r4 = resid(v4), t4 = resid(r4);
        const f32x2 r2 = resid(v2), t2 = resid(r2);
        const u32x4 P1 = pack6(v4, v2), P2 = pack6(r4, r2), P3 = pack6(t4, t2);
        u32x4 U0 = w[2 * 64], U1 = w[5 * 64];
        acc0 = mfma16(U0, P1, acc0); acc1 = mfma16(U1, P1, acc1);
        U0 = w[1 * 64]; U1 = w[4 * 64];
        acc0 = mfma16(U0, P2, acc0); acc1 = mfma16(U1, P2, acc1);
        acc0 = mfma16(U0, P1, acc0); acc1 = mfma16(U1, P1, acc1);
        U0 = w[0]; U1 = w[3 * 64];
        acc0 = mfma16(U0, P3, acc0); acc1 = mfma16(U1, P3, acc1);
        acc0 = mfma16(U0, P2, acc0); acc1 = mfma16(U1, P2, acc1);
        acc0 = mfma16(U0, P1, acc0); acc1 = mfma16(U1, P1, acc1);
    };
    float *w1t = carry_buf + C::CARRY_FLOATS;
    float *bt = w1t + 64 * 12;
    const f32x4 z4 = {0.f, 0.f, 0.f, 0.f};
    const f32x4 b2A = *(const f32x4 *)(bias2 + 4 * q), b2B = q < 2 ? *(const f32x4 *)(bias2 + 16 + 4 * q) : z4;

    const int cold_kx = W4 <= 16 ? 1 : 1 + (W4 - 16 + 14) / 15;
    const int tiles_x = COLD ? 1 : (W4 + 15) >> 4, tiles_y = (H4 + C::TH3 - 1) / C::TH3;
    const int strips = COLD ? n * tiles_y * cold_kx : n * tiles_y;
    const int D = tiles_x >= 3 ? 1 : 4 - tiles_x;
    int *ring = (int *)(bt + 64);
    float *lut = bt + 64 + 4;
    struct tpos { int tx, ty, img, ord, ls; };
    auto strip_pos = [&](int ord, int tx) {
        tpos p;
        if constexpr (COLD) {
            const int ls = (int)blockIdx.x + ord * (int)gridDim.x;
            const int sidx = ubd_xcd_tile(ls < strips ? ls : strips - 1, strips);
            const int rowi = (int)((unsigned)sidx / (unsigned)cold_kx);
            p.tx = sidx - rowi * cold_kx;
            p.ty = (int)((unsigned)rowi % (unsigned)tiles_y);
            p.img = (int)((unsigned)rowi / (unsigned)tiles_y);
            p.ord = ord; p.ls = ls;
            return p;
        }
        const int ls = __builtin_amdgcn_readfirstlane(ring[ord & 3]);
        const int sidx = ubd_xcd_tile(ls < strips ? ls : strips - 1, strips);
        p.ty = (int)((unsigned)sidx % (unsigned)tiles_y);
        p.img = (int)((unsigned)sidx / (unsigned)tiles_y);
        p.tx = tx; p.ord = ord; p.ls = ls;
        return p;
    };
    auto advance = [&](tpos p) {
        if (!COLD && p.tx + 1 < tiles_x) { ++p.tx; return p; }
        return strip_pos(p.ord + 1, 0);
    };
    auto xo3 = [&](const tpos &p) { return (COLD ? 15 : 16) * p.tx; };

    unsigned xreg[X::XREGS];
    constexpr int RWF = X::XW * CIN;
    const int e0_row = (int)threadIdx.x / RWF, e0_col = (int)threadIdx.x - e0_row * RWF;
    auto tile_interior = [&](tpos p) {
        const int iy0 = 4 * p.ty * C::TH3 - 5, ix0 = 4 * xo3(p) - 3;
        return (iy0 >= 0) && (ix0 >= 0) && (iy0 + X::XH <= H) && (ix0 + X::XW <= W);
    };
    auto load_x = [&](tpos p) {
        const int iy0 = 4 * p.ty * C::TH3 - 5, fx0 = (4 * xo3(p) - 3) * CIN, WC = W * CIN;
        const unsigned char *img8 = (const unsigned char *)xin + (size_t)p.img * H * WC * (IN_U8 ? 1 : 4);
        const bool interior = tile_interior(p);
        int pr = e0_row, pcf = e0_col;
#pragma unroll
        for (int k = 0; k < X::XREGS; ++k) {
            int gy = iy0 + pr, gf = fx0 + pcf;
            if (!interior) { gy = min(max(gy, 0), H - 1); gf = min(max(gf, 0), WC - 1); }
            else if (k == X::XREGS - 1) gy = min(gy, H - 1);
            const unsigned off = (unsigned)__umul24(gy, WC) + (unsigned)gf;
            if constexpr (IN_U8) xreg[k] = img8[off];
            else xreg[k] = ((const unsigned *)img8)[off];
            pr += C::NT / RWF; pcf += C::NT % RWF;
            if (pcf >= RWF) { pcf -= RWF; ++pr; }
        }
    };
    auto fix_border = [&](tpos p) {
        const int iy0 = 4 * p.ty * C::TH3 - 5, fx0 = (4 * xo3(p) - 3) * CIN, WC = W * CIN;
        int pr = e0_row, pcf = e0_col;
#pragma unroll
        for (int k = 0; k < X::XREGS; ++k) {
            const bool inside = (unsigned)(iy0 + pr) < (unsigned)H && (unsigned)(fx0 + pcf) < (unsigned)WC;
            xreg[k] = inside ? xreg[k] : (IN_U8 ? 0x100u : __builtin_bit_cast(unsigned, pre_sub));
            pr += C::NT / RWF; pcf += C::NT % RWF;
            if (pcf >= RWF) { pcf -= RWF; ++pr; }
        }
    };

    const unsigned lds_xp = ubd_lds_addr(xp);
    auto dma_x = [&](tpos p) {
        const int iy0 = 4 * p.ty * C::TH3 - 5, fx0 = (4 * xo3(p) - 4) * CIN, WC = W * CIN;
        __amdgpu_buffer_rsrc_t rsrc = __builtin_amdgcn_make_buffer_rsrc((void *)((const char *)xin + (size_t)p.img * H * WC * 4), 0,
                                                                        (int)((unsigned)H * WC * 4u), 0x00020000);
        unsigned off0 = (unsigned)lane * 16u;
        off0 = (unsigned)(fx0 + 4 * lane) < (unsigned)WC ? off0 : 0x80000000u;
        if (lane < X::XCH) {
#pragma unroll
            for (int k = 0; k < (X::XH + C::NW - 1) / C::NW; ++k) {
                const int row = k * C::NW + wid;
                if (row >= X::XH) break;
                const int term = ((iy0 + row) * WC + fx0) * 4;
                ubd_blds16(rsrc, (unsigned)term + off0, lds_xp + (unsigned)(row * X::XS * 4));
            }
        }
    };

    constexpr int UPW = 4;
    int u_rc[UPW];
#pragma unroll
    for (int k = 0; k < UPW; ++k) {
        const int u = wid >= 4 ? (wid - 4) + 4 * k : (k < 2 ? 16 + wid + 4 * k : X::UNITS);
        const int p = u * 16 + i;
        const bool live = u < X::UNITS && p < X::NPIX;
        const int ar = (live ? p : 0) / X::AC, ac = (live ? p : 0) - ar * X::AC + 1;
        u_rc[k] = live ? ((ar << 8) | ac) : -1;
    }
    auto u_rc_tile = [&](int k) {
        int rc = u_rc[k];
        if constexpr (!PLAIN) asm volatile("" : "+v"(rc));
        return rc;
    };
    const int qc = q < CIN ? q : CIN - 1;
    const int half = wid & 1, rg = wid >> 1;
    const int rb = rg == 0 ? 0 : 2 * rg + 1, rw = rg == 0 ? 3 : 2;
    const int pos = 1 + 16 * half + i;
    int ro4[3], ro2[3];
#pragma unroll
    for (int kx = 0; kx < 3; ++kx) {
        const int pcol = pos + kx;
        ro4[kx] = (rb * C::PW + pcol) * UBD_C + 4 * s123_slot(q, pcol);
        ro2[kx] = (rb * C::PW + pcol) * UBD_C + 4 * s123_slot(4 + (q >> 1), pcol) + 2 * (q & 1);
    }
    const int l2w = (rb * C::LC + pos) * C::LP + 4 * q;
    const int l2r = (2 * (wid & 3) * C::LC + 2 * i) * C::LP;

    if (!COLD && threadIdx.x == 0) {
        const bool had_job = (int)blockIdx.x < njob;
#pragma unroll
        for (int j = 0; j < 3; ++j) ring[j] = had_job ? ticket_ls(t0_early + j) : (int)blockIdx.x * D + j;
    }
    __syncthreads();
    tpos cur = strip_pos(0, 0);
    S123_BLOCK_STAMP(3);
    auto check_out = [&]() {
        if constexpr (COLD) return;
        __syncthreads();
        if (threadIdx.x == 0) {
            const int left = __hip_atomic_fetch_add(ticket + 16, 1, __ATOMIC_RELAXED, __HIP_MEMORY_SCOPE_AGENT);
            if (left == (int)gridDim.x - 1) {
                __hip_atomic_store(ticket, 0, __ATOMIC_RELAXED, __HIP_MEMORY_SCOPE_AGENT);
                __hip_atomic_store(ticket + 16, 0, __ATOMIC_RELAXED, __HIP_MEMORY_SCOPE_AGENT);
            }
        }
    };
    if (cur.ls >= strips) { S123_BLOCK_STAMP(2); check_out(); return; }
    tpos nx1 = advance(cur);
    int pending = 0;
#define S123_STAMP(k) UBD_STAMP(it < 16, (((size_t)blockIdx.x * 8 + wid) * 16 + it) * 8 + (k))
    auto convert_x = [&](tpos p) {
        const bool plain = !IN_U8 && pre_sub == 0.f && pre_div == 1.f;
        if (!tile_interior(p)) fix_border(p);
        int pr = e0_row, pcf = e0_col;
#pragma unroll
        for (int k = 0; k < X::XREGS; ++k) {
            const int e = k * C::NT + (int)threadIdx.x;
            if (e < X::XE) {
                float *dst = xp + pr * X::XS + CIN + pcf;
                if constexpr (IN_U8) *dst = xreg[k] > 255u ? 0.f : lut[xreg[k] & 255u];
                else *dst = plain ? __builtin_bit_cast(float, xreg[k]) : (__builtin_bit_cast(float, xreg[k]) - pre_sub) / pre_div;
            }
            pr += C::NT / RWF; pcf += C::NT % RWF;
            if (pcf >= RWF) { pcf -= RWF; ++pr; }
        }
    };
    auto l1_taps = [&](int k, float (&tap)[9]) {
        const int rck = u_rc_tile(k);
        const int rc0 = rck < 0 ? 1 : rck;
        const int ar0 = rc0 >> 8, ac0 = rc0 & 255;
        const int u_rd = (2 * ar0) * X::XS + (2 * (ac0 - 1) + 1) * CIN + qc;
#pragma unroll
        for (int ky = 0; ky < 3; ++ky)
#pragma unroll
            for (int kx = 0; kx < 3; ++kx) tap[ky * 3 + kx] = xp[u_rd + ky * X::XS + kx * CIN];
    };
    auto l1_finish = [&](tpos p, auto nunits, auto &tap, int k0) {
        constexpr int NU = decltype(nunits)::value;
        const int A0y = 2 * p.ty * C::TH3 - 2, A0x = 2 * xo3(p) - 2;
        float dwk1[9], pwf1[2];
        {
            const f32x4 wa = *(const f32x4 *)(w1t + lane * 12), wb = *(const f32x4 *)(w1t + lane * 12 + 4), wc = *(const f32x4 *)(w1t + lane * 12 + 8);
            dwk1[0] = wa[0]; dwk1[1] = wa[1]; dwk1[2] = wa[2]; dwk1[3] = wa[3]; dwk1[4] = wb[0]; dwk1[5] = wb[1]; dwk1[6] = wb[2]; dwk1[7] = wb[3];
            dwk1[8] = wc[0]; pwf1[0] = wc[1]; pwf1[1] = wc[2];
        }
        const f32x4 b1A = *(const f32x4 *)(bt + 4 * q), b1B = *(const f32x4 *)(bt + 16 + 4 * q);
        float dv[NU];
#pragma unroll
        for (int k = 0; k < NU; ++k) dv[k] = 0.f;
#pragma unroll
        for (int t = 0; t < 9; ++t)
#pragma unroll
            for (int k = 0; k < NU; ++k) dv[k] = fmaf(tap[k][t], dwk1[t], dv[k]);
        f32x4 acc0[NU], acc1[NU];
#pragma unroll
        for (int k = 0; k < NU; ++k) {
            acc0[k] = __builtin_amdgcn_mfma_f32_16x16x4f32(pwf1[0], dv[k], b1A, 0, 0, 0);
            acc1[k] = __builtin_amdgcn_mfma_f32_16x16x4f32(pwf1[1], dv[k], b1B, 0, 0, 0);
        }
#pragma unroll
        for (int k = 0; k < NU; ++k) {
            const int rc = u_rc_tile(k0 + k);
            const int ar = rc >> 8, ac = rc & 255;
            const bool inside = rc >= 0 && (unsigned)(A0y + ar) < (unsigned)H2 && (unsigned)(A0x + ac) < (unsigned)W2;
            const float cap = inside ? __builtin_inff() : 0.f;
#pragma unroll
            for (int r = 0; r < 4; ++r) { acc0[k][r] = ubd_relu_cap(acc0[k][r], cap); acc1[k][r] = ubd_relu_cap(acc1[k][r], cap); }
            if (rc >= 0) {
                float *dst = a1p + (ar * C::PW + ac) * UBD_C + 4 * s123_slot(q, ac);
                *(f32x4 *)dst = acc0[k];
                if (q < 2) {
                    *(f32x4 *)(a1p + (ar * C::PW + ac) * UBD_C + 4 * s123_slot(4 + q, ac)) = acc1[k];
                }
            }
        }
    };
    auto phase0b = [&](tpos p) {
        if (wid < 4) {
            float tap[2][9];
            l1_taps(0, tap[0]); l1_taps(1, tap[1]);
            l1_finish(p, std::integral_constant<int, 2>{}, tap, 0);
        } else {
            float tap[2][9];
            l1_taps(0, tap[0]); l1_taps(1, tap[1]);
            l1_finish(p, std::integral_constant<int, 2>{}, tap, 0);
            l1_taps(2, tap[0]); l1_taps(3, tap[1]);
            l1_finish(p, std::integral_constant<int, 2>{}, tap, 2);
        }
    };

    if constexpr (PLAIN) dma_x(cur); else load_x(cur);
    {
        static_assert(64 * 12 <= 2 * C::NT && 2 * X::PWS_U32 / 3 == 2 * C::NT && C::W3DW_FLOATS <= C::NT, "table entries per thread");
        auto w1_entry = [&](int e) {
            const int ln = e / 12, k = e - ln * 12;
            return k < 9 ? frag1[UBD_SEP_FRAG_FLOATS + (k * 6) * 64 + ln] : (k < 11 ? frag1[(k - 9) * 64 + ln] : 0.f);
        };
        auto pw_weight = [&](int e, int s) {
            const int nt = (e >> 8) & 1, ln = (e >> 2) & 63, lq = ln >> 4, li = ln & 15;
            const int ch = s < 4 ? 4 * lq + s : 16 + 2 * lq + (s - 4);
            return s < 6 ? ((e >> 9) ? frag3 : frag2)[((ch % 6) * 2 + nt) * 64 + 16 * (ch / 6) + li] : 0.f;
        };
        auto pw_store = [&](int e, float lo, float hi) {
            unsigned bl[3], bh[3];
            split3_bits(lo, bl); split3_bits(hi, bh);
            unsigned *dst = pws + (e >> 9) * X::PWS_U32 + (((e >> 8) & 1) * 3 * 64 + ((e >> 2) & 63)) * 4 + (e & 3);
#pragma unroll
            for (int pc = 0; pc < 3; ++pc) dst[pc * 64 * 4] = (bl[pc] >> 16) | bh[pc];
        };
        auto w3dw_entry = [&](int e) {
            const int lq = e / 72, r = e - lq * 72, t = r >> 3, s = r & 7;
            const int ch = s < 4 ? 4 * lq + s : 16 + 2 * lq + (s - 4);
            return s < 6 ? frag3[UBD_SEP_FRAG_FLOATS + (t * 6 + ch % 6) * 64 + 16 * (ch / 6)] : 0.f;
        };
        const int t = (int)threadIdx.x;
        const int e1 = t + C::NT < 64 * 12 ? t + C::NT : t, ed = t < C::W3DW_FLOATS ? t : 0;
        const float v0 = w1_entry(t), v1 = w1_entry(e1), v4 = w3dw_entry(ed);
        const int d0 = 2 * (t & 3), d1 = d0 + 1;
        const float p0 = pw_weight(t, d0), p1 = pw_weight(t, d1), p2 = pw_weight(t + C::NT, d0), p3 = pw_weight(t + C::NT, d1);
        const float v5 = (t & 31) < UBD_C ? (t < 32 ? bias1 : bias3)[t & 31] : 0.f;
        w1t[t] = v0; w1t[e1] = v1; w3dw[ed] = v4;
        pw_store(t, p0, p1); pw_store(t + C::NT, p2, p3);
        if (t < 64) bt[t] = v5;
        if constexpr (IN_U8) { if (t < 256) lut[t] = ((float)t - pre_sub) / pre_div; }
    }
    if constexpr (PLAIN) asm volatile("s_waitcnt vmcnt(0)" ::: "memory");
    else {
        if constexpr (IN_U8) __syncthreads();
        convert_x(cur);
    }
    __syncthreads();
    S123_BLOCK_STAMP(29);
    phase0b(cur);
    __syncthreads();
    S123_BLOCK_STAMP(30);
    for (int it = 0;; ++it) {
        S123_STAMP(0);
        const bool new_strip = !COLD && cur.tx == 0;
        if (new_strip) S123_BLOCK_STAMP(4 + cur.ord);
        if (new_strip && threadIdx.x == 0) pending = __hip_atomic_fetch_add(ticket, 1, __ATOMIC_RELAXED, __HIP_MEMORY_SCOPE_AGENT);
        const int img = cur.img, oy0 = cur.ty * C::TH3, ox0 = xo3(cur);
        const bool has_next = nx1.ls < strips;
        const int R0 = 2 * oy0 - 1, C0 = 2 * ox0 - 1;
        if (has_next) { if constexpr (PLAIN) dma_x(nx1); else load_x(nx1); }
        if (wid == C::NW - 1 && lane < C::LR * 6) {
            const int row = lane / 6, ch4 = lane - row * 6;
            f32x4 v = z4;
            if (!COLD && cur.tx > 0) v = *(const f32x4 *)(carry_buf + (((it + 1) & 1) * C::LR + row) * C::LP + 4 * ch4);
            *(f32x4 *)(l2 + (row * C::LC) * C::LP + 4 * ch4) = v;
        }
        S123_STAMP(1);

        const bool mask_needed = (R0 < 0) || (R0 + C::LR > H2) || (C0 + C::LC > W2);
        {
            float dwv[3][6];
#pragma unroll
            for (int o = 0; o < 3; ++o)
#pragma unroll
                for (int s = 0; s < 6; ++s) dwv[o][s] = 0.f;
#pragma unroll
            for (int yy = 0; yy < 5; ++yy) {
                if (yy < rw + 2) {
                    f32x4 v4[3];
                    f32x2 v2[3];
#pragma unroll
                    for (int kx = 0; kx < 3; ++kx) {
                        v4[kx] = *(const f32x4 *)(a1p + ro4[kx] + yy * (C::PW * UBD_C));
                        v2[kx] = *(const f32x2 *)(a1p + ro2[kx] + yy * (C::PW * UBD_C));
                    }
#pragma unroll
                    for (int o = 0; o < 3; ++o) {
                        const int ky = yy - o;
                        if (ky < 0 || ky > 2) continue;
#pragma unroll
                        for (int kx = 0; kx < 3; ++kx) {
                            const int t = ky * 3 + kx;
                            dwv[o][0] = fmaf(v4[kx][0], dwk2[t][0], dwv[o][0]);
                            dwv[o][1] = fmaf(v4[kx][1], dwk2[t][1], dwv[o][1]);
                            dwv[o][2] = fmaf(v4[kx][2], dwk2[t][2], dwv[o][2]);
                            dwv[o][3] = fmaf(v4[kx][3], dwk2[t][3], dwv[o][3]);
                            dwv[o][4] = fmaf(v2[kx][0], dwk2[t][4], dwv[o][4]);
                            dwv[o][5] = fmaf(v2[kx][1], dwk2[t][5], dwv[o][5]);
                        }
                    }
                    if (yy >= 2) {
                        const int o = yy - 2;
                        f32x4 acc0 = b2A, acc1 = b2B;
                        pw_split(pws, (f32x4){dwv[o][0], dwv[o][1], dwv[o][2], dwv[o][3]}, (f32x2){dwv[o][4], dwv[o][5]}, acc0, acc1);
                        float cap = __builtin_inff();
                        if (mask_needed) {
                            const bool ok = (unsigned)(C0 + pos) < (unsigned)W2 && (unsigned)(R0 + rb + o) < (unsigned)H2;
                            cap = ok ? cap : 0.f;
                        }
#pragma unroll
                        for (int r = 0; r < 4; ++r) { acc0[r] = ubd_relu_cap(acc0[r], cap); acc1[r] = ubd_relu_cap(acc1[r], cap); }
                        float *dst = l2 + l2w + o * (C::LC * C::LP);
                        *(f32x4 *)dst = acc0;
                        if (q < 2) *(f32x4 *)(dst + 16) = acc1;
                        if (half == 1 && i == 15) {
                            float *cd = carry_buf + ((it & 1) * C::LR + rb + o) * C::LP + 4 * q;
                            *(f32x4 *)cd = acc0;
                            if (q < 2) *(f32x4 *)(cd + 16) = acc1;
                        }
                    }
                }
            }
        }
        S123_STAMP(2);
        if (has_next) {
            if constexpr (PLAIN) asm volatile("s_waitcnt vmcnt(0)" ::: "memory");
            else convert_x(nx1);
        }
        S123_STAMP(3);
        __syncthreads();
        S123_STAMP(4);

        if (wid < 4) {
            const int oy = oy0 + wid;
            float dv[6] = {0.f, 0.f, 0.f, 0.f, 0.f, 0.f};
#pragma unroll
            for (int ky = 0; ky < 3; ++ky)
#pragma unroll
                for (int kx = 0; kx < 3; ++kx) {
                    const float *p = l2 + l2r + (ky * C::LC + kx) * C::LP;
                    const f32x4 v4 = *(const f32x4 *)(p + 4 * q);
                    const f32x2 v2 = *(const f32x2 *)(p + 16 + 2 * q);
                    const float *wt = w3dw + (q * 9 + ky * 3 + kx) * 8;
                    const f32x4 w4 = *(const f32x4 *)wt;
                    const f32x2 w2 = *(const f32x2 *)(wt + 4);
                    dv[0] = fmaf(v4[0], w4[0], dv[0]); dv[1] = fmaf(v4[1], w4[1], dv[1]);
                    dv[2] = fmaf(v4[2], w4[2], dv[2]); dv[3] = fmaf(v4[3], w4[3], dv[3]);
                    dv[4] = fmaf(v2[0], w2[0], dv[4]); dv[5] = fmaf(v2[1], w2[1], dv[5]);
                }
            f32x4 acc0 = *(const f32x4 *)(bt + 32 + 4 * q), acc1 = *(const f32x4 *)(bt + 48 + 4 * q);
            pw_split(pws + X::PWS_U32, (f32x4){dv[0], dv[1], dv[2], dv[3]}, (f32x2){dv[4], dv[5]}, acc0, acc1);
            store_tile_relu_nb(y, ((size_t)img * H4 + oy) * W4, ox0, oy < H4 ? W4 : 0, lane, acc0, acc1, COLD && cur.tx > 0 && i == 0, a3_l2p);
            S123_STAMP(5);
            if (!has_next) break;
            float tap[2][9];
            l1_taps(0, tap[0]); l1_taps(1, tap[1]);
            l1_finish(nx1, std::integral_constant<int, 2>{}, tap, 0);
        } else {
            S123_STAMP(5);
            if (!has_next) break;
            float tap[2][9];
            l1_taps(0, tap[0]); l1_taps(1, tap[1]);
            l1_finish(nx1, std::integral_constant<int, 2>{}, tap, 0);
            l1_taps(2, tap[0]); l1_taps(3, tap[1]);
            l1_finish(nx1, std::integral_constant<int, 2>{}, tap, 2);
        }
        S123_STAMP(6);
        if (new_strip && threadIdx.x == 0) ring[(cur.ord + D) & 3] = ticket_ls(pending);
        __syncthreads();
        S123_STAMP(7);
        cur = nx1;
        nx1 = advance(nx1);
    }
    S123_BLOCK_STAMP(2);
    check_out();
}
```

### ubdvss_amd/csrc/stem_plan.h

```cpp
#pragma once

enum {
    UBD_STEM_SEPARATE = 0,
    UBD_STEM_FUSED23 = 1,
    UBD_STEM_FUSED123 = 2,
    UBD_STEM_COLD123 = 3,
};

enum ubd_stem_form {
    UBD_STEM_FORM_SEPARATE,
    UBD_STEM_FORM_L1_STEM23,
    UBD_STEM_FORM_STRIPS,
    UBD_STEM_FORM_COLD,
};

#define UBD_STEM_STRIP_ROWS 4

struct ubd_stem_plan {
    ubd_stem_form form;
    long strips;
    bool job_without_strips;
};

static inline ubd_stem_plan ubd_plan_stem(int setting, bool forced, bool fml, int num_cus, int n, int H, bool inference, bool job)
{
    ubd_stem_plan p;
    p.strips = (long)n * ((H / 4 + UBD_STEM_STRIP_ROWS - 1) / UBD_STEM_STRIP_ROWS);
    const bool big = forced || p.strips >= 2L * num_cus;
    if (inference && big && setting == UBD_STEM_FUSED123 && fml) p.form = UBD_STEM_FORM_STRIPS;
    else if (inference && !job && fml && (setting == UBD_STEM_COLD123 || (setting == UBD_STEM_FUSED123 && !forced))) p.form = UBD_STEM_FORM_COLD;
    else if (inference && big && setting != UBD_STEM_SEPARATE) p.form = UBD_STEM_FORM_L1_STEM23;
    else p.form = UBD_STEM_FORM_SEPARATE;
    p.job_without_strips = job && p.form != UBD_STEM_FORM_STRIPS;
    return p;
}
```

Measured before the change: 100,800 images/s.

## Split the stem's last strips into column tiles to balance the postprocess tail

When a fused postprocess job shares the strip-form stem kernel, the last few strip rows are reserved and handed out as individual column tiles from a second atomic ticket counter. Blocks finish their strips, then pick tail tiles at finer granularity, so that blocks that are busy with CCL jobs do not leave the stem's end unbalanced. This adds a templated TAIL variant, an extra ticket slot that is reset at kernel exit, and generic tile-position lambdas. The cost is more code paths, overlapping halo work on the narrower tail tiles, and extra atomics.

```diff
diff --git a/ubdvss_amd/csrc/api.hip b/ubdvss_amd/csrc/api.hip
--- a/ubdvss_amd/csrc/api.hip
+++ b/ubdvss_amd/csrc/api.hip
@@ -114,6 +114,7 @@
     h->num_cus = prop.multiProcessorCount;
     h->use_wino = h->wino_x6 = h->chain_reduce = 1;
     h->fuse_stem = cfg->fml_compatible != 0 ? UBD_STEM_FUSED123 : UBD_STEM_SEPARATE;
+    h->stem_cold_tail = -1;
     for (const env_switch &sw : ENV_SWITCHES) {
         const char *e = getenv(sw.name);
         if (!e) continue;
@@ -121,6 +122,7 @@
         if (sw.value == NUMBER) { if (atoi(e) > 0) *field = atoi(e); }
         else if (sw.value == ANY || strcmp(e, sw.value) == 0) *field = sw.set;
     }
+    { const char *s = getenv("UBD_STEM_COLD_TAIL"); if (s && *s >= '0' && *s <= '9') h->stem_cold_tail = atoi(s); }
     { const char *s = getenv("UBD_STEM"); if (s && strcmp(s, "cold123") == 0 && cfg->fml_compatible != 0) { h->fuse_stem = UBD_STEM_COLD123; h->fuse_force = 1; } }
     size_t off = 0;
     int cin = cfg->c_in;
diff --git a/ubdvss_amd/csrc/common.h b/ubdvss_amd/csrc/common.h
--- a/ubdvss_amd/csrc/common.h
+++ b/ubdvss_amd/csrc/common.h
@@ -22,6 +22,7 @@
     size_t n_params;
     int num_cus;
     int pp_lds_attr_set;
+    int stem_cold_tail;
     int fuse_force;
     int split_headbwd;
     int no_pair_dilbwd;
diff --git a/ubdvss_amd/csrc/forward.hip b/ubdvss_amd/csrc/forward.hip
--- a/ubdvss_amd/csrc/forward.hip
+++ b/ubdvss_amd/csrc/forward.hip
@@ -642,7 +642,7 @@
 template <bool COLD>
 static void launch_stem123(const ubd_handle *h, const float *params, const void *images, bool u8, float *a3, const float *sf0, const float *sf1,
                            const float *sf2, int n, int H, int W, float sc, float sh, long units, int *ticket, const pp_lds_args *job, int a3_l2p,
-                           hipStream_t st)
+                           int tail_rows, hipStream_t st)
 {
     const int H2 = H / 2, W2 = W / 2, H4 = H / 4, W4 = W / 4;
     const int grid = units < h->num_cus ? (int)units : h->num_cus;
@@ -653,13 +653,28 @@
     const bool plain = ubd_pixels_by_lds_dma(!u8, sc, sh, H, W, h->cfg.c_in, 1ull << 30, images);
     ubd_dispatch_input(h->cfg.c_in, u8, [&](auto cin, auto in_u8) {
         auto launch = [&](auto pl) {
-            hipLaunchKernelGGL((stem123_kernel<decltype(cin)::value, decltype(in_u8)::value, decltype(pl)::value, COLD>), dim3(grid), dim3(s23_cfg::NT), 0, st,
-                               images, a3, sf0, b0, sf1, b1, sf2, b2, n, H, W, H2, W2, H4, W4, sc, sh, ticket, pj, a3_l2p
-                               UBD_STAMP_ARG(COLD ? "" : "stem123"));
+            ubd_dispatch_bool(!COLD && tail_rows > 0, [&](auto tail) {
+                if constexpr (COLD && decltype(tail)::value) return;
+                else hipLaunchKernelGGL((stem123_kernel<decltype(cin)::value, decltype(in_u8)::value, decltype(pl)::value, COLD, decltype(tail)::value>),
+                                        dim3(grid), dim3(s23_cfg::NT), 0, st,
+                                        images, a3, sf0, b0, sf1, b1, sf2, b2, n, H, W, H2, W2, H4, W4, sc, sh, ticket, pj, a3_l2p, tail_rows
+                                        UBD_STAMP_ARG(COLD ? "" : "stem123"));
+            });
         };
         if constexpr (decltype(in_u8)::value == 0) { if (plain) return launch(ubd_int<1>{}); }
         launch(ubd_int<0>{});
     });
+}
+
+static ubd_stem_plan plan_stem_of(const ubd_handle *h, int n, int H, int W, bool inference, int job_maps)
+{
+    return ubd_plan_stem(h->fuse_stem, h->fuse_force != 0, h->cfg.fml_compatible != 0, h->num_cus, n, H, inference, job_maps >= 0, W,
+                         job_maps > 0 ? job_maps : 0, h->stem_cold_tail);
+}
+extern "C" int ubd_stem_tail_rows(const ubd_handle *h, int n, int height, int width, int job_maps)
+{
+    if (!h || h->cfg.dtype != UBD_F32 || n <= 0 || height <= 0 || width <= 0) return 0;
+    return plan_stem_of(h, n, height, width, true, job_maps).tail_rows;
 }
 
 int ubd_forward_impl(ubd_handle *h, const float *params, const void *images, int in_dtype, int preprocessing,
@@ -689,7 +704,7 @@
     const int u8 = in_dtype == UBD_IN_U8;
     float *cur = (float *)(ws + L.off_acts[0]);
     static_assert(UBD_STEM_STRIP_ROWS == s23_cfg::TH3, "stem_plan.h counts the strips the stem kernels walk");
-    const ubd_stem_plan plan = ubd_plan_stem(h->fuse_stem, h->fuse_force != 0, h->cfg.fml_compatible != 0, h->num_cus, n, H, inference, pp_job != nullptr);
+    const ubd_stem_plan plan = plan_stem_of(h, n, H, W, inference, pp_job ? pp_job->n : -1);
     UBD_REQUIRE(!plan.job_without_strips, "ubd_forward: a postprocess job needs the fused stem kernel (internal error)");
     const bool one_kernel = plan.form == UBD_STEM_FORM_STRIPS || plan.form == UBD_STEM_FORM_COLD;
     static const int phase_lay[UBD_NUM_DIL + 1] = {2, 4, 1, 1, 1, 2, 1};
@@ -698,9 +713,9 @@
     int *ticket = (int *)(ws + L.off_tickets);
     if (plan.form == UBD_STEM_FORM_COLD)
         launch_stem123<true>(h, params, images, u8, cur, sf0, sf1, sf2, n, H, W, sc, sh, plan.strips * (W4 <= 16 ? 1 : 1 + (W4 - 16 + 14) / 15),
-                             ticket, nullptr, a3_l2p, st);
+                             ticket, nullptr, a3_l2p, 0, st);
     else if (plan.form == UBD_STEM_FORM_STRIPS)
-        launch_stem123<false>(h, params, images, u8, cur, sf0, sf1, sf2, n, H, W, sc, sh, plan.strips, ticket, pp_job, a3_l2p, st);
+        launch_stem123<false>(h, params, images, u8, cur, sf0, sf1, sf2, n, H, W, sc, sh, plan.strips, ticket, pp_job, a3_l2p, plan.tail_rows, st);
     else if (h->cfg.c_in == 1)
         launch_sep<1, 2>(h, images, u8, a1, sf0, params + h->off_sep_b[0], n, H, W, H2, W2, pad_s2, sc, sh, st);
     else
diff --git a/ubdvss_amd/csrc/stem123.h b/ubdvss_amd/csrc/stem123.h
--- a/ubdvss_amd/csrc/stem123.h
+++ b/ubdvss_amd/csrc/stem123.h
@@ -26,14 +26,17 @@
     static_assert(XCH <= 64 && (A1_FLOATS % 4) == 0 && (B::L2_FLOATS % 4) == 0, "patch rows are single 16-byte-aligned DMA pieces");
 };
 
-template <int CIN, int IN_U8, int PLAIN, bool COLD = false>
+template <bool CW> struct s123_tpos { static constexpr bool cold = CW; int tx, ty, img, ord, ls; };
+
+template <int CIN, int IN_U8, int PLAIN, bool COLD = false, bool TAIL = false>
 __global__ __launch_bounds__(s23_cfg::NT, 1) void stem123_kernel(const void *__restrict__ xin, float *__restrict__ y,
                                                                 const float *__restrict__ frag1, const float *__restrict__ bias1,
                                                                 const float *__restrict__ frag2, const float *__restrict__ bias2,
                                                                 const float *__restrict__ frag3, const float *__restrict__ bias3,
                                                                 int n, int H, int W, int H2, int W2, int H4, int W4,
                                                                 float pre_sub, float pre_div, int *__restrict__ ticket, pp_lds_args pj,
-                                                                int a3_l2p
+                                                                int a3_l2p ,
+                                                                int tail_rows
                                                                 UBD_STAMP_PARAM)
 {
     using C = s23_cfg;
@@ -96,9 +99,13 @@
     const int D = tiles_x >= 3 ? 1 : 4 - tiles_x;
     int *ring = (int *)(bt + 64);
     float *lut = bt + 64 + 4;
-    struct tpos { int tx, ty, img, ord, ls; };
-    auto strip_pos = [&](int ord, int tx) {
-        tpos p;
+    const int strips_end = TAIL ? strips - tail_rows : strips;
+    static_assert(!(COLD && TAIL), "the tail belongs to the strip form");
+    const int tail_tiles = TAIL ? tail_rows * cold_kx : 0;
+    using cold_c = std::bool_constant<true>;
+    auto pos_limit = [&](auto cw) { return COLD ? strips : (decltype(cw)::value ? tail_tiles : strips_end); };
+    auto strip_pos = [&](auto cw, int ord, int tx) {
+        s123_tpos<decltype(cw)::value> p;
         if constexpr (COLD) {
             const int ls = (int)blockIdx.x + ord * (int)gridDim.x;
             const int sidx = ubd_xcd_tile(ls < strips ? ls : strips - 1, strips);
@@ -108,28 +115,39 @@
             p.img = (int)((unsigned)rowi / (unsigned)tiles_y);
             p.ord = ord; p.ls = ls;
             return p;
-        }
-        const int ls = __builtin_amdgcn_readfirstlane(ring[ord & 3]);
-        const int sidx = ubd_xcd_tile(ls < strips ? ls : strips - 1, strips);
-        p.ty = (int)((unsigned)sidx % (unsigned)tiles_y);
-        p.img = (int)((unsigned)sidx / (unsigned)tiles_y);
-        p.tx = tx; p.ord = ord; p.ls = ls;
-        return p;
-    };
-    auto advance = [&](tpos p) {
-        if (!COLD && p.tx + 1 < tiles_x) { ++p.tx; return p; }
-        return strip_pos(p.ord + 1, 0);
-    };
-    auto xo3 = [&](const tpos &p) { return (COLD ? 15 : 16) * p.tx; };
+        } else if constexpr (decltype(cw)::value) {
+            const int tk = __builtin_amdgcn_readfirstlane(ring[ord & 3]);
+            const int tc = tk < tail_tiles ? tk : tail_tiles - 1;
+            const int rel = (int)((unsigned)tc / (unsigned)cold_kx);
+            const int sidx = ubd_xcd_tile(strips_end + rel, strips);
+            p.tx = tc - rel * cold_kx;
+            p.ty = (int)((unsigned)sidx % (unsigned)tiles_y);
+            p.img = (int)((unsigned)sidx / (unsigned)tiles_y);
+            p.ord = ord; p.ls = tk;
+            return p;
+        } else {
+            const int ls = __builtin_amdgcn_readfirstlane(ring[ord & 3]);
+            const int sidx = ubd_xcd_tile(ls < strips ? ls : strips - 1, strips);
+            p.ty = (int)((unsigned)sidx % (unsigned)tiles_y);
+            p.img = (int)((unsigned)sidx / (unsigned)tiles_y);
+            p.tx = tx; p.ord = ord; p.ls = ls;
+            return p;
+        }
+    };
+    auto advance = [&](auto p) {
+        if (!decltype(p)::cold && p.tx + 1 < tiles_x) { ++p.tx; return p; }
+        return strip_pos(std::bool_constant<decltype(p)::cold>{}, p.ord + 1, 0);
+    };
+    auto xo3 = [&](auto p) { return (decltype(p)::cold ? 15 : 16) * p.tx; };
 
     unsigned xreg[X::XREGS];
     constexpr int RWF = X::XW * CIN;
     const int e0_row = (int)threadIdx.x / RWF, e0_col = (int)threadIdx.x - e0_row * RWF;
-    auto tile_interior = [&](tpos p) {
+    auto tile_interior = [&](auto p) {
         const int iy0 = 4 * p.ty * C::TH3 - 5, ix0 = 4 * xo3(p) - 3;
         return (iy0 >= 0) && (ix0 >= 0) && (iy0 + X::XH <= H) && (ix0 + X::XW <= W);
     };
-    auto load_x = [&](tpos p) {
+    auto load_x = [&](auto p) {
         const int iy0 = 4 * p.ty * C::TH3 - 5, fx0 = (4 * xo3(p) - 3) * CIN, WC = W * CIN;
         const unsigned char *img8 = (const unsigned char *)xin + (size_t)p.img * H * WC * (IN_U8 ? 1 : 4);
         const bool interior = tile_interior(p);
@@ -146,7 +164,7 @@
             if (pcf >= RWF) { pcf -= RWF; ++pr; }
         }
     };
-    auto fix_border = [&](tpos p) {
+    auto fix_border = [&](auto p) {
         const int iy0 = 4 * p.ty * C::TH3 - 5, fx0 = (4 * xo3(p) - 3) * CIN, WC = W * CIN;
         int pr = e0_row, pcf = e0_col;
 #pragma unroll
@@ -159,7 +177,7 @@
     };
 
     const unsigned lds_xp = ubd_lds_addr(xp);
-    auto dma_x = [&](tpos p) {
+    auto dma_x = [&](auto p) {
         const int iy0 = 4 * p.ty * C::TH3 - 5, fx0 = (4 * xo3(p) - 4) * CIN, WC = W * CIN;
         __amdgpu_buffer_rsrc_t rsrc = __builtin_amdgcn_make_buffer_rsrc((void *)((const char *)xin + (size_t)p.img * H * WC * 4), 0,
                                                                         (int)((unsigned)H * WC * 4u), 0x00020000);
@@ -211,24 +229,25 @@
         for (int j = 0; j < 3; ++j) ring[j] = had_job ? ticket_ls(t0_early + j) : (int)blockIdx.x * D + j;
     }
     __syncthreads();
-    tpos cur = strip_pos(0, 0);
+    const auto first = strip_pos(std::bool_constant<COLD>{}, 0, 0);
     S123_BLOCK_STAMP(3);
+    int pending = 0;
     auto check_out = [&]() {
         if constexpr (COLD) return;
+        asm volatile("" :: "v"(pending) : "memory");
         __syncthreads();
         if (threadIdx.x == 0) {
             const int left = __hip_atomic_fetch_add(ticket + 16, 1, __ATOMIC_RELAXED, __HIP_MEMORY_SCOPE_AGENT);
             if (left == (int)gridDim.x - 1) {
                 __hip_atomic_store(ticket, 0, __ATOMIC_RELAXED, __HIP_MEMORY_SCOPE_AGENT);
                 __hip_atomic_store(ticket + 16, 0, __ATOMIC_RELAXED, __HIP_MEMORY_SCOPE_AGENT);
-            }
-        }
-    };
-    if (cur.ls >= strips) { S123_BLOCK_STAMP(2); check_out(); return; }
-    tpos nx1 = advance(cur);
-    int pending = 0;
-#define S123_STAMP(k) UBD_STAMP(it < 16, (((size_t)blockIdx.x * 8 + wid) * 16 + it) * 8 + (k))
-    auto convert_x = [&](tpos p) {
+                __hip_atomic_store(ticket + 32, 0, __ATOMIC_RELAXED, __HIP_MEMORY_SCOPE_AGENT);
+            }
+        }
+    };
+    if (first.ls >= pos_limit(std::bool_constant<COLD>{}) && tail_tiles == 0) { S123_BLOCK_STAMP(2); check_out(); return; }
+#define S123_STAMP(k) UBD_STAMP(tile_stamps && it < 16, (((size_t)blockIdx.x * 8 + wid) * 16 + it) * 8 + (k))
+    auto convert_x = [&](auto p) {
         const bool plain = !IN_U8 && pre_sub == 0.f && pre_div == 1.f;
         if (!tile_interior(p)) fix_border(p);
         int pr = e0_row, pcf = e0_col;
@@ -254,7 +273,7 @@
 #pragma unroll
             for (int kx = 0; kx < 3; ++kx) tap[ky * 3 + kx] = xp[u_rd + ky * X::XS + kx * CIN];
     };
-    auto l1_finish = [&](tpos p, auto nunits, auto &tap, int k0) {
+    auto l1_finish = [&](auto p, auto nunits, auto &tap, int k0) {
         constexpr int NU = decltype(nunits)::value;
         const int A0y = 2 * p.ty * C::TH3 - 2, A0x = 2 * xo3(p) - 2;
         float dwk1[9], pwf1[2];
@@ -294,7 +313,7 @@
             }
         }
     };
-    auto phase0b = [&](tpos p) {
+    auto phase0b = [&](auto p) {
         if (wid < 4) {
             float tap[2][9];
             l1_taps(0, tap[0]); l1_taps(1, tap[1]);
@@ -308,8 +327,7 @@
         }
     };
 
-    if constexpr (PLAIN) dma_x(cur); else load_x(cur);
-    {
+    auto fill_tables = [&]() {
         static_assert(64 * 12 <= 2 * C::NT && 2 * X::PWS_U32 / 3 == 2 * C::NT && C::W3DW_FLOATS <= C::NT, "table entries per thread");
         auto w1_entry = [&](int e) {
             const int ln = e / 12, k = e - ln * 12;
@@ -342,138 +360,163 @@
         pw_store(t, p0, p1); pw_store(t + C::NT, p2, p3);
         if (t < 64) bt[t] = v5;
         if constexpr (IN_U8) { if (t < 256) lut[t] = ((float)t - pre_sub) / pre_div; }
-    }
-    if constexpr (PLAIN) asm volatile("s_waitcnt vmcnt(0)" ::: "memory");
-    else {
-        if constexpr (IN_U8) __syncthreads();
-        convert_x(cur);
-    }
-    __syncthreads();
-    S123_BLOCK_STAMP(29);
-    phase0b(cur);
-    __syncthreads();
-    S123_BLOCK_STAMP(30);
-    for (int it = 0;; ++it) {
-        S123_STAMP(0);
-        const bool new_strip = !COLD && cur.tx == 0;
-        if (new_strip) S123_BLOCK_STAMP(4 + cur.ord);
-        if (new_strip && threadIdx.x == 0) pending = __hip_atomic_fetch_add(ticket, 1, __ATOMIC_RELAXED, __HIP_MEMORY_SCOPE_AGENT);
-        const int img = cur.img, oy0 = cur.ty * C::TH3, ox0 = xo3(cur);
-        const bool has_next = nx1.ls < strips;
-        const int R0 = 2 * oy0 - 1, C0 = 2 * ox0 - 1;
-        if (has_next) { if constexpr (PLAIN) dma_x(nx1); else load_x(nx1); }
-        if (wid == C::NW - 1 && lane < C::LR * 6) {
-            const int row = lane / 6, ch4 = lane - row * 6;
-            f32x4 v = z4;
-            if (!COLD && cur.tx > 0) v = *(const f32x4 *)(carry_buf + (((it + 1) & 1) * C::LR + row) * C::LP + 4 * ch4);
-            *(f32x4 *)(l2 + (row * C::LC) * C::LP + 4 * ch4) = v;
-        }
-        S123_STAMP(1);
-
-        const bool mask_needed = (R0 < 0) || (R0 + C::LR > H2) || (C0 + C::LC > W2);
-        {
-            float dwv[3][6];
-#pragma unroll
-            for (int o = 0; o < 3; ++o)
-#pragma unroll
-                for (int s = 0; s < 6; ++s) dwv[o][s] = 0.f;
-#pragma unroll
-            for (int yy = 0; yy < 5; ++yy) {
-                if (yy < rw + 2) {
-                    f32x4 v4[3];
-                    f32x2 v2[3];
-#pragma unroll
-                    for (int kx = 0; kx < 3; ++kx) {
-                        v4[kx] = *(const f32x4 *)(a1p + ro4[kx] + yy * (C::PW * UBD_C));
-                        v2[kx] = *(const f32x2 *)(a1p + ro2[kx] + yy * (C::PW * UBD_C));
-                    }
-#pragma unroll
-                    for (int o = 0; o < 3; ++o) {
-                        const int ky = yy - o;
-                        if (ky < 0 || ky > 2) continue;
+    };
+    auto walk = [&](auto cur, bool tables_needed) {
+        constexpr bool CW = decltype(cur)::cold;
+        constexpr bool tile_stamps = COLD || !CW;
+        (void)tile_stamps;
+        const int limit = pos_limit(std::bool_constant<CW>{});
+        auto nx1 = advance(cur);
+        if constexpr (PLAIN) dma_x(cur); else load_x(cur);
+        if (tables_needed) fill_tables();
+        if constexpr (PLAIN) asm volatile("s_waitcnt vmcnt(0)" ::: "memory");
+        else {
+            if constexpr (IN_U8) __syncthreads();
+            convert_x(cur);
+        }
+        __syncthreads();
+        if constexpr (tile_stamps) S123_BLOCK_STAMP(29);
+        phase0b(cur);
+        __syncthreads();
+        if constexpr (tile_stamps) S123_BLOCK_STAMP(30);
+        for (int it = 0;; ++it) {
+            S123_STAMP(0);
+            const bool new_strip = COLD ? false : (CW || cur.tx == 0);
+            if (new_strip && !CW) S123_BLOCK_STAMP(4 + cur.ord);
+            if (new_strip && threadIdx.x == 0) pending = __hip_atomic_fetch_add(ticket + (CW ? 32 : 0), 1, __ATOMIC_RELAXED, __HIP_MEMORY_SCOPE_AGENT);
+            const int img = cur.img, oy0 = cur.ty * C::TH3, ox0 = xo3(cur);
+            const bool has_next = nx1.ls < limit;
+            const int R0 = 2 * oy0 - 1, C0 = 2 * ox0 - 1;
+            if (has_next) { if constexpr (PLAIN) dma_x(nx1); else load_x(nx1); }
+            if (wid == C::NW - 1 && lane < C::LR * 6) {
+                const int row = lane / 6, ch4 = lane - row * 6;
+                f32x4 v = z4;
+                if (!CW && cur.tx > 0) v = *(const f32x4 *)(carry_buf + (((it + 1) & 1) * C::LR + row) * C::LP + 4 * ch4);
+                *(f32x4 *)(l2 + (row * C::LC) * C::LP + 4 * ch4) = v;
+            }
+            S123_STAMP(1);
+
+            const bool mask_needed = (R0 < 0) || (R0 + C::LR > H2) || (C0 + C::LC > W2);
+            {
+                float dwv[3][6];
+#pragma unroll
+                for (int o = 0; o < 3; ++o)
+#pragma unroll
+                    for (int s = 0; s < 6; ++s) dwv[o][s] = 0.f;
+#pragma unroll
+                for (int yy = 0; yy < 5; ++yy) {
+                    if (yy < rw + 2) {
+                        f32x4 v4[3];
+                        f32x2 v2[3];
 #pragma unroll
                         for (int kx = 0; kx < 3; ++kx) {
-                            const int t = ky * 3 + kx;
-                            dwv[o][0] = fmaf(v4[kx][0], dwk2[t][0], dwv[o][0]);
-                            dwv[o][1] = fmaf(v4[kx][1], dwk2[t][1], dwv[o][1]);
-                            dwv[o][2] = fmaf(v4[kx][2], dwk2[t][2], dwv[o][2]);
-                            dwv[o][3] = fmaf(v4[kx][3], dwk2[t][3], dwv[o][3]);
-                            dwv[o][4] = fmaf(v2[kx][0], dwk2[t][4], dwv[o][4]);
-                            dwv[o][5] = fmaf(v2[kx][1], dwk2[t][5], dwv[o][5]);
+                            v4[kx] = *(const f32x4 *)(a1p + ro4[kx] + yy * (C::PW * UBD_C));
+                            v2[kx] = *(const f32x2 *)(a1p + ro2[kx] + yy * (C::PW * UBD_C));
                         }
-                    }
-                    if (yy >= 2) {
-                        const int o = yy - 2;
-                        f32x4 acc0 = b2A, acc1 = b2B;
-                        pw_split(pws, (f32x4){dwv[o][0], dwv[o][1], dwv[o][2], dwv[o][3]}, (f32x2){dwv[o][4], dwv[o][5]}, acc0, acc1);
-                        float cap = __builtin_inff();
-                        if (mask_needed) {
-                            const bool ok = (unsigned)(C0 + pos) < (unsigned)W2 && (unsigned)(R0 + rb + o) < (unsigned)H2;
-                            cap = ok ? cap : 0.f;
+#pragma unroll
+                        for (int o = 0; o < 3; ++o) {
+                            const int ky = yy - o;
+                            if (ky < 0 || ky > 2) continue;
+#pragma unroll
+                            for (int kx = 0; kx < 3; ++kx) {
+                                const int t = ky * 3 + kx;
+                                dwv[o][0] = fmaf(v4[kx][0], dwk2[t][0], dwv[o][0]);
+                                dwv[o][1] = fmaf(v4[kx][1], dwk2[t][1], dwv[o][1]);
+                                dwv[o][2] = fmaf(v4[kx][2], dwk2[t][2], dwv[o][2]);
+                                dwv[o][3] = fmaf(v4[kx][3], dwk2[t][3], dwv[o][3]);
+                                dwv[o][4] = fmaf(v2[kx][0], dwk2[t][4], dwv[o][4]);
+                                dwv[o][5] = fmaf(v2[kx][1], dwk2[t][5], dwv[o][5]);
+                            }
                         }
-#pragma unroll
-                        for (int r = 0; r < 4; ++r) { acc0[r] = ubd_relu_cap(acc0[r], cap); acc1[r] = ubd_relu_cap(acc1[r], cap); }
-                        float *dst = l2 + l2w + o * (C::LC * C::LP);
-                        *(f32x4 *)dst = acc0;
-                        if (q < 2) *(f32x4 *)(dst + 16) = acc1;
-                        if (half == 1 && i == 15) {
-                            float *cd = carry_buf + ((it & 1) * C::LR + rb + o) * C::LP + 4 * q;
-                            *(f32x4 *)cd = acc0;
-                            if (q < 2) *(f32x4 *)(cd + 16) = acc1;
+                        if (yy >= 2) {
+                            const int o = yy - 2;
+                            f32x4 acc0 = b2A, acc1 = b2B;
+                            pw_split(pws, (f32x4){dwv[o][0], dwv[o][1], dwv[o][2], dwv[o][3]}, (f32x2){dwv[o][4], dwv[o][5]}, acc0, acc1);
+                            float cap = __builtin_inff();
+                            if (mask_needed) {
+                                const bool ok = (unsigned)(C0 + pos) < (unsigned)W2 && (unsigned)(R0 + rb + o) < (unsigned)H2;
+                                cap = ok ? cap : 0.f;
+                            }
+#pragma unroll
+                            for (int r = 0; r < 4; ++r) { acc0[r] = ubd_relu_cap(acc0[r], cap); acc1[r] = ubd_relu_cap(acc1[r], cap); }
+                            float *dst = l2 + l2w + o * (C::LC * C::LP);
+                            *(f32x4 *)dst = acc0;
+                            if (q < 2) *(f32x4 *)(dst + 16) = acc1;
+                            if (half == 1 && i == 15) {
+                                float *cd = carry_buf + ((it & 1) * C::LR + rb + o) * C::LP + 4 * q;
+                                *(f32x4 *)cd = acc0;
+                                if (q < 2) *(f32x4 *)(cd + 16) = acc1;
+                            }
                         }
                     }
                 }
             }
-        }
-        S123_STAMP(2);
-        if (has_next) {
-            if constexpr (PLAIN) asm volatile("s_waitcnt vmcnt(0)" ::: "memory");
-            else convert_x(nx1);
-        }
-        S123_STAMP(3);
-        __syncthreads();
-        S123_STAMP(4);
-
-        if (wid < 4) {
-            const int oy = oy0 + wid;
-            float dv[6] = {0.f, 0.f, 0.f, 0.f, 0.f, 0.f};
-#pragma unroll
-            for (int ky = 0; ky < 3; ++ky)
-#pragma unroll
-                for (int kx = 0; kx < 3; ++kx) {
-                    const float *p = l2 + l2r + (ky * C::LC + kx) * C::LP;
-                    const f32x4 v4 = *(const f32x4 *)(p + 4 * q);
-                    const f32x2 v2 = *(const f32x2 *)(p + 16 + 2 * q);
-                    const float *wt = w3dw + (q * 9 + ky * 3 + kx) * 8;
-                    const f32x4 w4 = *(const f32x4 *)wt;
-                    const f32x2 w2 = *(const f32x2 *)(wt + 4);
-                    dv[0] = fmaf(v4[0], w4[0], dv[0]); dv[1] = fmaf(v4[1], w4[1], dv[1]);
-                    dv[2] = fmaf(v4[2], w4[2], dv[2]); dv[3] = fmaf(v4[3], w4[3], dv[3]);
-                    dv[4] = fmaf(v2[0], w2[0], dv[4]); dv[5] = fmaf(v2[1], w2[1], dv[5]);
-                }
-            f32x4 acc0 = *(const f32x4 *)(bt + 32 + 4 * q), acc1 = *(const f32x4 *)(bt + 48 + 4 * q);
-            pw_split(pws + X::PWS_U32, (f32x4){dv[0], dv[1], dv[2], dv[3]}, (f32x2){dv[4], dv[5]}, acc0, acc1);
-            store_tile_relu_nb(y, ((size_t)img * H4 + oy) * W4, ox0, oy < H4 ? W4 : 0, lane, acc0, acc1, COLD && cur.tx > 0 && i == 0, a3_l2p);
-            S123_STAMP(5);
-            if (!has_next) break;
-            float tap[2][9];
-            l1_taps(0, tap[0]); l1_taps(1, tap[1]);
-            l1_finish(nx1, std::integral_constant<int, 2>{}, tap, 0);
-        } else {
-            S123_STAMP(5);
-            if (!has_next) break;
-            float tap[2][9];
-            l1_taps(0, tap[0]); l1_taps(1, tap[1]);
-            l1_finish(nx1, std::integral_constant<int, 2>{}, tap, 0);
-            l1_taps(2, tap[0]); l1_taps(3, tap[1]);
-            l1_finish(nx1, std::integral_constant<int, 2>{}, tap, 2);
-        }
-        S123_STAMP(6);
-        if (new_strip && threadIdx.x == 0) ring[(cur.ord + D) & 3] = ticket_ls(pending);
-        __syncthreads();
-        S123_STAMP(7);
-        cur = nx1;
-        nx1 = advance(nx1);
+            S123_STAMP(2);
+            if (has_next) {
+                if constexpr (PLAIN) asm volatile("s_waitcnt vmcnt(0)" ::: "memory");
+                else convert_x(nx1);
+            }
+            S123_STAMP(3);
+            __syncthreads();
+            S123_STAMP(4);
+
+            if (wid < 4) {
+                const int oy = oy0 + wid;
+                float dv[6] = {0.f, 0.f, 0.f, 0.f, 0.f, 0.f};
+#pragma unroll
+                for (int ky = 0; ky < 3; ++ky)
+#pragma unroll
+                    for (int kx = 0; kx < 3; ++kx) {
+                        const float *p = l2 + l2r + (ky * C::LC + kx) * C::LP;
+                        const f32x4 v4 = *(const f32x4 *)(p + 4 * q);
+                        const f32x2 v2 = *(const f32x2 *)(p + 16 + 2 * q);
+                        const float *wt = w3dw + (q * 9 + ky * 3 + kx) * 8;
+                        const f32x4 w4 = *(const f32x4 *)wt;
+                        const f32x2 w2 = *(const f32x2 *)(wt + 4);
+                        dv[0] = fmaf(v4[0], w4[0], dv[0]); dv[1] = fmaf(v4[1], w4[1], dv[1]);
+                        dv[2] = fmaf(v4[2], w4[2], dv[2]); dv[3] = fmaf(v4[3], w4[3], dv[3]);
+                        dv[4] = fmaf(v2[0], w2[0], dv[4]); dv[5] = fmaf(v2[1], w2[1], dv[5]);
+                    }
+                f32x4 acc0 = *(const f32x4 *)(bt + 32 + 4 * q), acc1 = *(const f32x4 *)(bt + 48 + 4 * q);
+                pw_split(pws + X::PWS_U32, (f32x4){dv[0], dv[1], dv[2], dv[3]}, (f32x2){dv[4], dv[5]}, acc0, acc1);
+                store_tile_relu_nb(y, ((size_t)img * H4 + oy) * W4, ox0, oy < H4 ? W4 : 0, lane, acc0, acc1, CW && cur.tx > 0 && i == 0, a3_l2p);
+                S123_STAMP(5);
+                if (!has_next) break;
+                float tap[2][9];
+                l1_taps(0, tap[0]); l1_taps(1, tap[1]);
+                l1_finish(nx1, std::integral_constant<int, 2>{}, tap, 0);
+            } else {
+                S123_STAMP(5);
+                if (!has_next) break;
+                float tap[2][9];
+                l1_taps(0, tap[0]); l1_taps(1, tap[1]);
+                l1_finish(nx1, std::integral_constant<int, 2>{}, tap, 0);
+                l1_taps(2, tap[0]); l1_taps(3, tap[1]);
+                l1_finish(nx1, std::integral_constant<int, 2>{}, tap, 2);
+            }
+            S123_STAMP(6);
+            if (new_strip && threadIdx.x == 0) ring[(cur.ord + (CW ? 3 : D)) & 3] = CW ? pending : ticket_ls(pending);
+            __syncthreads();
+            S123_STAMP(7);
+            cur = nx1;
+            nx1 = advance(nx1);
+        }
+    };
+    if (first.ls < pos_limit(std::bool_constant<COLD>{})) walk(first, true);
+    else if constexpr (TAIL) fill_tables();
+    if constexpr (TAIL) {
+        if (tail_tiles > 0) {
+            __syncthreads();
+            S123_BLOCK_STAMP(31);
+            if (threadIdx.x == 0) {
+                const int t0 = __hip_atomic_fetch_add(ticket + 32, 3, __ATOMIC_RELAXED, __HIP_MEMORY_SCOPE_AGENT);
+#pragma unroll
+                for (int j = 0; j < 3; ++j) ring[j] = t0 + j;
+            }
+            __syncthreads();
+            const auto ct = strip_pos(cold_c{}, 0, 0);
+            if (ct.ls < tail_tiles) walk(ct, false);
+        }
     }
     S123_BLOCK_STAMP(2);
     check_out();
diff --git a/ubdvss_amd/csrc/stem_plan.h b/ubdvss_amd/csrc/stem_plan.h
--- a/ubdvss_amd/csrc/stem_plan.h
+++ b/ubdvss_amd/csrc/stem_plan.h
@@ -20,9 +20,13 @@
     ubd_stem_form form;
     long strips;
     bool job_without_strips;
+    int tail_rows;
 };
 
-static inline ubd_stem_plan ubd_plan_stem(int setting, bool forced, bool fml, int num_cus, int n, int H, bool inference, bool job)
+#define UBD_STEM_TAIL_ROWS_PER_JOB_BLOCK 4
+
+static inline ubd_stem_plan ubd_plan_stem(int setting, bool forced, bool fml, int num_cus, int n, int H, bool inference, bool job,
+                                          int W = 0, int job_maps = 0, int tail_override = -1)
 {
     ubd_stem_plan p;
     p.strips = (long)n * ((H / 4 + UBD_STEM_STRIP_ROWS - 1) / UBD_STEM_STRIP_ROWS);
@@ -32,5 +36,14 @@
     else if (inference && big && setting != UBD_STEM_SEPARATE) p.form = UBD_STEM_FORM_L1_STEM23;
     else p.form = UBD_STEM_FORM_SEPARATE;
     p.job_without_strips = job && p.form != UBD_STEM_FORM_STRIPS;
+    p.tail_rows = 0;
+    if (p.form == UBD_STEM_FORM_STRIPS && job && job_maps > 0 && W > 0) {
+        const long grid = p.strips < num_cus ? p.strips : num_cus;
+        const int tiles_x = (W / 4 + 15) / 16, D = tiles_x >= 3 ? 1 : 4 - tiles_x;
+        const long job_blocks = job_maps < grid ? job_maps : grid;
+        const long want = tail_override >= 0 ? tail_override : (long)UBD_STEM_TAIL_ROWS_PER_JOB_BLOCK * job_blocks;
+        const long room = p.strips - grid * D;
+        p.tail_rows = (int)(want < room ? want : (room > 0 ? room : 0));
+    }
     return p;
 }
```

Measured after the change: 102,700 images/s, median of 6. 1.9% higher.
